# montyhall/bot7

Measured on NVIDIA B200. Metric: EI candidates scored/s at N=4096, S=32 hypers, higher is better.
Workload: dtype f64

## Files before the change

bot7_b200/csrc/api.cu:

```cuda
#include <math.h>
#include <stdarg.h>
#include <cmath>
#include <stdio.h>
#include <string.h>
#include <stdlib.h>

#include <algorithm>

#include "b7_internal.h"

static thread_local char g_err[512] = "";

void b7_set_error(const char* fmt, ...) {
  va_list ap;
  va_start(ap, fmt);
  vsnprintf(g_err, sizeof(g_err), fmt, ap);
  va_end(ap);
}

int b7_score_grid_size(b7_ctx* ctx, int64_t M);

namespace {

constexpr int kParStride = B7_MAX_DIMS + 4;
constexpr double kLog2Pi = 1.83787706640934548356;

constexpr size_t kCacheMin = (size_t)1 << 20;

void cache_flush(b7_ctx* ctx) {
  for (const b7_ctx::Block& b : ctx->cache) cudaFreeAsync(b.p, ctx->stream);
  ctx->cache.clear();
  ctx->cache_bytes = 0;
}

int dev_alloc_bytes(b7_ctx* ctx, void** p, size_t bytes) {
  *p = nullptr;
  bytes = (bytes + 255) / 256 * 256;
  if (bytes == 0) bytes = 256;
  if (bytes >= kCacheMin)
    for (size_t i = 0; i < ctx->cache.size(); ++i)
      if (ctx->cache[i].bytes == bytes) {
        *p = ctx->cache[i].p;
        ctx->cache_bytes -= bytes;
        ctx->cache[i] = ctx->cache.back();
        ctx->cache.pop_back();
        ctx->live[*p] = bytes;
        return 0;
      }
  cudaError_t e = cudaMallocFromPoolAsync(p, bytes, ctx->pool, ctx->stream);
  if (e != cudaSuccess && !ctx->cache.empty()) {
    cudaGetLastError();
    cache_flush(ctx);
    cudaStreamSynchronize(ctx->stream);
    cudaMemPoolTrimTo(ctx->pool, 0);
    e = cudaMallocFromPoolAsync(p, bytes, ctx->pool, ctx->stream);
  }
  if (e != cudaSuccess) {
    cudaGetLastError();
    b7_set_error("device allocation of %zu bytes failed: %s", bytes, cudaGetErrorString(e));
    return B7_ERR_NOMEM;
  }
  if (bytes >= kCacheMin) ctx->live[*p] = bytes;
  return 0;
}

template <typename T>
int dev_alloc(b7_ctx* ctx, T** p, size_t count) { return dev_alloc_bytes(ctx, (void**)p, (count ? count : 1) * sizeof(T)); }

inline void dev_free(b7_ctx* ctx, void* p) {
  if (!p) return;
  auto it = ctx->live.find(p);
  if (it != ctx->live.end()) {
    const size_t bytes = it->second;
    ctx->live.erase(it);
    if (ctx->cache_bytes + bytes <= ctx->cache_cap) {
      ctx->cache.push_back({p, bytes});
      ctx->cache_bytes += bytes;
      return;
    }
  }
  cudaFreeAsync(p, ctx->stream);
}

int grow(b7_ctx* ctx, double** p, size_t* have, size_t need_bytes) {
  if (*have >= need_bytes) return 0;
  dev_free(ctx, *p);
  *p = nullptr; *have = 0;
  B7_CHECK(dev_alloc(ctx, p, need_bytes / sizeof(double) + 1));
  *have = need_bytes;
  return 0;
}

inline int64_t pad128(int64_t n) { return (n + 127) / 128 * 128; }

inline int64_t panel_rows(b7_ctx* ctx, int Np = 4096) {
  const int64_t base = (int64_t)ctx->sm_count * 128;
  const int64_t f = Np >= 4096 ? 1 : std::min<int64_t>(8, 4096 / std::max(Np, 128));
  return base * f;
}

int sync_removed(b7_grid* g) {
  if (!g->removed_dirty) return 0;
  int64_t n = (int64_t)g->removed.size();
  if (n > g->removed_cap) {
    dev_free(g->ctx, g->removed_dev);
    g->removed_cap = std::max<int64_t>(256, 2 * n);
    B7_CHECK(dev_alloc(g->ctx, &g->removed_dev, (size_t)g->removed_cap));
  }
  if (n > 0)
    B7_CUDA(cudaMemcpyAsync(g->removed_dev, g->removed.data(), n * sizeof(int64_t), cudaMemcpyHostToDevice, g->ctx->stream));
  g->removed_dirty = false;
  return 0;
}

__device__ __forceinline__ long long tiled_index(int Np, int row, int k) {
  return ((long long)(row >> 7) * (Np >> 4) + (k >> 4)) * 2048 + ((k >> 2) & 3) * 512 + (row & 127) * 4 + (k & 3);
}

__global__ void frob_rows_kernel(const double* __restrict__ A, int Np, int N, double* __restrict__ out) {
  __shared__ double sh[256];
  double s = 0.0;
  const int row = blockIdx.x;
  for (int k = threadIdx.x; k <= row; k += blockDim.x) {
    const double v = A[tiled_index(Np, row, k)];
    s += (k < row ? 2.0 : 1.0) * v * v;
  }
  sh[threadIdx.x] = s;
  __syncthreads();
  for (int o = 128; o > 0; o >>= 1) {
    if (threadIdx.x < o) sh[threadIdx.x] += sh[threadIdx.x + o];
    __syncthreads();
  }
  if (threadIdx.x == 0) out[blockIdx.x] = sh[0];
}

__global__ void identity_kernel(double* __restrict__ A, int Np) {
  long long e = (long long)blockIdx.x * blockDim.x + threadIdx.x;
  if (e < (long long)Np * Np) { const int row = (int)(e / Np), k = (int)(e % Np); A[tiled_index(Np, row, k)] = (row == k) ? 1.0 : 0.0; }
}

int upload_residual(b7_gp* gp, int s, const std::vector<double>& yh) {
  std::vector<double> r((size_t)gp->Np, 0.0);
  const double m = gp->par_host[(size_t)s * kParStride + B7_MAX_DIMS + 2];
  for (int i = 0; i < gp->N; ++i) r[i] = yh[i] - m;
  B7_CUDA(cudaMemcpyAsync(gp->beta + (size_t)s * gp->Np, r.data(), gp->Np * sizeof(double), cudaMemcpyHostToDevice, gp->ctx->stream));
  B7_CUDA(cudaStreamSynchronize(gp->ctx->stream));
  return 0;
}

int build_kxx(b7_gp* gp, int s0, int count) {
  b7_ctx* ctx = gp->ctx;
  StageTimer t(ctx, ST_KBUILD);
  B7_CHECK(b7_launch_cov_batched(ctx, gp->kernel, gp->X, gp->N, gp->Np, gp->d, gp->Xt, gp->N, gp->Np,
                                 gp->par + (size_t)s0 * kParStride, kParStride, gp->fac + (size_t)s0 * gp->Np * gp->Np,
                                 (int64_t)gp->Np * gp->Np, count, true, true));
  t.stop(1);
  return 0;
}

int factor(b7_gp* gp, int s0, int count) {
  b7_ctx* ctx = gp->ctx;
  StageTimer t(ctx, ST_POTRF);
  int64_t before = ctx->launches;
  B7_CHECK(b7_launch_potrf(gp, s0, count));
  t.stop((int)(ctx->launches - before));
  return 0;
}

}

int b7_pool_alloc(b7_ctx* ctx, void** p, size_t bytes) {
  char* q = nullptr;
  int rc = dev_alloc(ctx, &q, bytes);
  *p = q;
  return rc;
}
void b7_pool_free(b7_ctx* ctx, void* p) { dev_free(ctx, p); }


extern "C" {

int b7_version(void) { return 100; }
const char* b7_last_error(void) { return g_err; }

int b7_device_count(void) {
  int n = 0;
  if (cudaGetDeviceCount(&n) != cudaSuccess) return 0;
  return n;
}

int b7_init(int device, b7_ctx** out) {
  if (!out) { b7_set_error("b7_init: out is null"); return B7_ERR_ARG; }
  *out = nullptr;
  int n = 0;
  cudaError_t e = cudaGetDeviceCount(&n);
  if (e != cudaSuccess || n == 0) {
    b7_set_error("b7_init: no CUDA device (%s); this library has no CPU path", e == cudaSuccess ? "count 0" : cudaGetErrorString(e));
    return B7_ERR_CUDA;
  }
  if (device < 0 || device >= n) { b7_set_error("b7_init: device %d out of range [0,%d)", device, n); return B7_ERR_ARG; }
  B7_CUDA(cudaSetDevice(device));
  b7_ctx* ctx = new b7_ctx();
  ctx->device = device;
  cudaDeviceProp p;
  B7_CUDA(cudaGetDeviceProperties(&p, device));
  ctx->sm_count = p.multiProcessorCount;
  if (p.major < 10) { b7_set_error("b7_init: device is sm_%d%d, this build is sm_100a only", p.major, p.minor); delete ctx; return B7_ERR_CUDA; }
  int prio_lo = 0, prio_hi = 0;
  B7_CUDA(cudaDeviceGetStreamPriorityRange(&prio_lo, &prio_hi));
  B7_CUDA(cudaStreamCreateWithPriority(&ctx->stream, cudaStreamNonBlocking, prio_hi));
  B7_CUDA(cudaStreamCreateWithPriority(&ctx->stream2, cudaStreamNonBlocking, prio_lo));
  B7_CUDA(cudaEventCreateWithFlags(&ctx->evA, cudaEventDisableTiming));
  B7_CUDA(cudaEventCreateWithFlags(&ctx->evB, cudaEventDisableTiming));
  B7_CUDA(cudaStreamCreateWithPriority(&ctx->stream3, cudaStreamNonBlocking, (prio_hi + prio_lo) / 2));
  B7_CUDA(cudaEventCreateWithFlags(&ctx->evS, cudaEventDisableTiming));
  B7_CUDA(cudaEventCreateWithFlags(&ctx->evS1, cudaEventDisableTiming));
  for (int i = 0; i < 2; ++i) {
    B7_CUDA(cudaEventCreateWithFlags(&ctx->evK[i], cudaEventDisableTiming));
    B7_CUDA(cudaEventCreateWithFlags(&ctx->evP[i], cudaEventDisableTiming));
  }
  { const char* e = getenv("B7_KSTAR_OVERLAP"); ctx->kstar_overlap = !(e && e[0] == '0'); }
  cudaMemPoolProps props = {};
  props.allocType = cudaMemAllocationTypePinned;
  props.handleTypes = cudaMemHandleTypeNone;
  props.location.type = cudaMemLocationTypeDevice;
  props.location.id = device;
  B7_CUDA(cudaMemPoolCreate(&ctx->pool, &props));
  unsigned long long keep = ~0ULL;
  B7_CUDA(cudaMemPoolSetAttribute(ctx->pool, cudaMemPoolAttrReleaseThreshold, &keep));
  {
    size_t free_b = 0, total_b = 0;
    B7_CUDA(cudaMemGetInfo(&free_b, &total_b));
    const char* e = getenv("B7_CACHE_FRACTION");
    const double frac = e ? atof(e) : 1.0 / 3.0;
    ctx->cache_cap = (size_t)((frac < 0.0 ? 0.0 : (frac > 0.9 ? 0.9 : frac)) * (double)total_b);
  }
  { const char* e = getenv("B7_POSTERIOR_I8"); ctx->use_i8 = !(e && e[0] == '0'); }
  { const char* e = getenv("B7_POTRF_I8"); ctx->potrf_i8 = !(e && e[0] == '0'); }
  { const char* e = getenv("B7_TRTRI_I8"); ctx->trtri_i8 = !(e && e[0] == '0'); }
  { const char* e = getenv("B7_POST_PAIR"); ctx->post_pair = !(e && e[0] == '0') && ctx->sm_count >= 2; }
  B7_CUDA(cudaEventCreate(&ctx->ev0));
  B7_CUDA(cudaEventCreate(&ctx->ev1));
  B7_CUDA(cudaEventCreate(&ctx->tm0));
  B7_CUDA(cudaEventCreate(&ctx->tm1));
  *out = ctx;
  return 0;
}

void b7_shutdown(b7_ctx* ctx) {
  if (!ctx) return;
  cudaSetDevice(ctx->device);
  cudaStreamSynchronize(ctx->stream);
  dev_free(ctx, ctx->ks);
  dev_free(ctx, ctx->moments);
  dev_free(ctx, ctx->xs_stage);
  dev_free(ctx, ctx->i8_partial);
  cache_flush(ctx);
  cudaStreamSynchronize(ctx->stream);
  cudaStreamSynchronize(ctx->stream2);
  cudaStreamSynchronize(ctx->stream3);
  cudaEventDestroy(ctx->evS);
  cudaEventDestroy(ctx->evS1);
  cudaStreamDestroy(ctx->stream3);
  cudaEventDestroy(ctx->evA);
  cudaEventDestroy(ctx->evB);
  for (int i = 0; i < 2; ++i) { cudaEventDestroy(ctx->evK[i]); cudaEventDestroy(ctx->evP[i]); }
  cudaStreamDestroy(ctx->stream2);
  cudaEventDestroy(ctx->ev0);
  cudaEventDestroy(ctx->ev1);
  cudaEventDestroy(ctx->tm0);
  cudaEventDestroy(ctx->tm1);
  cudaStreamDestroy(ctx->stream);
  if (ctx->pool) cudaMemPoolDestroy(ctx->pool);
  delete ctx;
}

int b7_sync(b7_ctx* ctx) {
  if (!ctx) return B7_ERR_ARG;
  B7_CUDA(cudaStreamSynchronize(ctx->stream));
  return 0;
}

int b7_set_posterior_path(b7_ctx* ctx, int path) {
  if (!ctx || (path != B7_PATH_FP64_DMMA && path != B7_PATH_INT8_OZAKI)) { b7_set_error("set_posterior_path: bad arguments"); return B7_ERR_ARG; }
  ctx->use_i8 = path == B7_PATH_INT8_OZAKI;
  return 0;
}
int b7_get_posterior_path(b7_ctx* ctx) { return ctx && ctx->use_i8 ? B7_PATH_INT8_OZAKI : B7_PATH_FP64_DMMA; }

int b7_timer_begin(b7_ctx* ctx) {
  if (!ctx) return B7_ERR_ARG;
  B7_CUDA(cudaSetDevice(ctx->device));
  B7_CUDA(cudaStreamSynchronize(ctx->stream));
  B7_CUDA(cudaEventRecord(ctx->tm0, ctx->stream));
  return 0;
}
int b7_timer_end(b7_ctx* ctx, double* ms) {
  if (!ctx || !ms) return B7_ERR_ARG;
  B7_CUDA(cudaEventRecord(ctx->tm1, ctx->stream));
  B7_CUDA(cudaEventSynchronize(ctx->tm1));
  float f = 0;
  B7_CUDA(cudaEventElapsedTime(&f, ctx->tm0, ctx->tm1));
  *ms = f;
  return 0;
}

int b7_set_profiling(b7_ctx* ctx, int on) { if (!ctx) return B7_ERR_ARG; ctx->profiling = on != 0; return 0; }
int b7_reset_stage_timers(b7_ctx* ctx) {
  if (!ctx) return B7_ERR_ARG;
  for (int i = 0; i < ST_COUNT; ++i) { ctx->stage_ms[i] = 0; ctx->stage_calls[i] = 0; }
  return 0;
}
int b7_last_stage_ms(b7_ctx* ctx, int stage, double* ms_total, int64_t* launches) {
  if (!ctx || stage < 0 || stage >= ST_COUNT) return B7_ERR_ARG;
  if (ms_total) *ms_total = ctx->stage_ms[stage];
  if (launches) *launches = ctx->stage_calls[stage];
  return 0;
}
int64_t b7_launch_count(b7_ctx* ctx) { return ctx ? ctx->launches : 0; }


int b7_sobol_directions(int dims, uint32_t* out) {
  if (dims < 1 || dims >= B7_MAX_DIMS || !out) { b7_set_error("sobol: dims must satisfy 1 <= dims < 40"); return B7_ERR_ARG; }
  b7_sobol_directions_host(dims, out);
  return 0;
}

int b7_sobol_generate(b7_ctx* ctx, int dims, int64_t first_seed, int64_t count, const double* mins,
                      const double* maxes, double* out_host, b7_grid** out_grid) {
  if (!ctx) return B7_ERR_ARG;
  if (out_grid) *out_grid = nullptr;
  if (dims < 1 || dims >= B7_MAX_DIMS) { b7_set_error("sobol: dims must satisfy 1 <= dims < 40"); return B7_ERR_ARG; }
  if (first_seed < 0) first_seed = 0;
  if (count < 0 || first_seed + count > (1LL << B7_SOBOL_BITS)) { b7_set_error("sobol: too many calls (seed range exceeds 2^30)"); return B7_ERR_ARG; }
  if ((mins == nullptr) != (maxes == nullptr)) { b7_set_error("sobol: one-sided rescaling is done by the host wrapper; pass both mins and maxes or neither"); return B7_ERR_ARG; }
  B7_CUDA(cudaSetDevice(ctx->device));
  double* dev = nullptr;
  B7_CHECK(dev_alloc(ctx, &dev, (size_t)count * dims));
  double *dmin = nullptr, *dscale = nullptr;
  if (mins) {
    double h[2 * B7_MAX_DIMS];
    for (int i = 0; i < dims; ++i) { h[i] = mins[i]; h[B7_MAX_DIMS + i] = maxes[i] + (-mins[i]); }
    B7_CHECK(dev_alloc(ctx, &dmin, 2 * B7_MAX_DIMS));
    dscale = dmin + B7_MAX_DIMS;
    B7_CUDA(cudaMemcpyAsync(dmin, h, sizeof(h), cudaMemcpyHostToDevice, ctx->stream));
    B7_CUDA(cudaStreamSynchronize(ctx->stream));
  }
  StageTimer t(ctx, ST_SOBOL);
  int rc = b7_launch_sobol(ctx, dims, first_seed, count, dmin, dscale, dev);
  t.stop(1);
  if (rc == 0 && out_host && count > 0) {
    cudaError_t e = cudaMemcpyAsync(out_host, dev, (size_t)count * dims * sizeof(double), cudaMemcpyDeviceToHost, ctx->stream);
    if (e != cudaSuccess) { b7_set_error("sobol D2H: %s", cudaGetErrorString(e)); rc = B7_ERR_CUDA; }
  }
  cudaError_t e = cudaStreamSynchronize(ctx->stream);
  if (rc == 0 && e != cudaSuccess) { b7_set_error("sobol: %s", cudaGetErrorString(e)); rc = B7_ERR_CUDA; }
  dev_free(ctx, dmin);
  if (rc != 0 || !out_grid) { dev_free(ctx, dev); return rc; }
  b7_grid* g = new b7_grid();
  g->ctx = ctx; g->rows = count; g->d = dims; g->X = dev;
  *out_grid = g;
  return 0;
}

int b7_grid_from_host(b7_ctx* ctx, const double* X, int64_t M, int d, b7_grid** out_grid) {
  if (!ctx || !out_grid || M < 0 || d < 1 || (M > 0 && !X)) { b7_set_error("grid_from_host: bad arguments"); return B7_ERR_ARG; }
  *out_grid = nullptr;
  B7_CUDA(cudaSetDevice(ctx->device));
  double* dev = nullptr;
  B7_CHECK(dev_alloc(ctx, &dev, (size_t)M * d));
  if (M > 0) {
    B7_CUDA(cudaMemcpyAsync(dev, X, (size_t)M * d * sizeof(double), cudaMemcpyHostToDevice, ctx->stream));
    B7_CUDA(cudaStreamSynchronize(ctx->stream));
  }
  b7_grid* g = new b7_grid();
  g->ctx = ctx; g->rows = M; g->d = d; g->X = dev;
  *out_grid = g;
  return 0;
}

int b7_grid_read(b7_grid* g, int64_t first_row, int64_t count, double* out_host) {
  if (!g || first_row < 0 || count < 0 || first_row + count > g->rows || (count > 0 && !out_host)) { b7_set_error("grid_read: range"); return B7_ERR_ARG; }
  B7_CUDA(cudaSetDevice(g->ctx->device));
  if (count == 0) return 0;
  B7_CUDA(cudaMemcpyAsync(out_host, g->X + first_row * g->d, (size_t)count * g->d * sizeof(double), cudaMemcpyDeviceToHost, g->ctx->stream));
  B7_CUDA(cudaStreamSynchronize(g->ctx->stream));
  return 0;
}

int64_t b7_grid_size(b7_grid* g) { return g ? g->rows - (int64_t)g->removed.size() : 0; }
int64_t b7_grid_rows(b7_grid* g) { return g ? g->rows : 0; }
int b7_grid_dims(b7_grid* g) { return g ? g->d : 0; }

static int64_t compacted_to_original(const b7_grid* g, int64_t c1) {
  int64_t r = c1 - 1;
  for (int64_t t : g->removed) {
    if (t <= r) ++r; else break;
  }
  return r;
}

int b7_grid_original_index(b7_grid* g, int64_t compacted_index, int64_t* original_index_1based) {
  if (!g || compacted_index < 1 || compacted_index > b7_grid_size(g)) { b7_set_error("grid: compacted index out of range"); return B7_ERR_ARG; }
  if (original_index_1based) *original_index_1based = compacted_to_original(g, compacted_index) + 1;
  return 0;
}

int b7_grid_remove(b7_grid* g, int64_t compacted_index, double* removed_row) {
  if (!g || compacted_index < 1 || compacted_index > b7_grid_size(g)) { b7_set_error("grid_remove: index out of range"); return B7_ERR_ARG; }
  int64_t r = compacted_to_original(g, compacted_index);
  if (removed_row) B7_CHECK(b7_grid_read(g, r, 1, removed_row));
  g->removed.insert(std::upper_bound(g->removed.begin(), g->removed.end(), r), r);
  g->removed_dirty = true;
  return 0;
}

void b7_grid_free(b7_grid* g) {
  if (!g) return;
  cudaSetDevice(g->ctx->device);
  dev_free(g->ctx, g->X);
  dev_free(g->ctx, g->removed_dev);
  delete g;
}


void b7_gp_free(b7_gp* gp) {
  if (!gp) return;
  cudaSetDevice(gp->ctx->device);
  cudaStreamSynchronize(gp->ctx->stream);
  void* ptrs[] = {gp->X, gp->Xt, gp->y, gp->par, gp->fac, gp->facS, gp->sigma, gp->dinv, gp->dinvT, gp->beta, gp->alpha, gp->tt, gp->logdet, gp->info, gp->meta_dev};
  for (void* p : ptrs) dev_free(gp->ctx, p);
  if (gp->potrf_graph) cudaGraphExecDestroy(gp->potrf_graph);
  delete gp;
}

int b7_gp_num_draws(b7_gp* gp) { return gp ? gp->S : 0; }
int b7_gp_num_obs(b7_gp* gp) { return gp ? gp->N : 0; }
int b7_gp_padded_n(b7_gp* gp) { return gp ? gp->Np : 0; }

static int gp_retry_draw(b7_gp* gp, int s, int first_info);

static void set_hypers_host(b7_gp* gp, const double* hyp) {
  const int d = gp->d, H = d + 3, S = gp->S;
  gp->par_host.assign((size_t)S * kParStride, 0.0);
  for (int s = 0; s < S; ++s) {
    const double* h = hyp + (size_t)s * H;
    double* p = gp->par_host.data() + (size_t)s * kParStride;
    for (int i = 0; i < d; ++i) p[i] = exp(-h[i]);
    const double sf2 = exp(2.0 * h[d]), sn2 = exp(2.0 * h[d + 1]);
    p[B7_MAX_DIMS] = sf2;
    p[B7_MAX_DIMS + 1] = sn2 + (gp->noiseless ? 1e-8 * sf2 : 0.0);
    p[B7_MAX_DIMS + 2] = h[d + 2];
    p[B7_MAX_DIMS + 3] = sn2;
  }
}

static void residuals_host(b7_gp* gp, const std::vector<double>& y, std::vector<double>& r) {
  r.assign((size_t)gp->S * gp->Np, 0.0);
  for (int s = 0; s < gp->S; ++s) {
    const double m = gp->par_host[(size_t)s * kParStride + B7_MAX_DIMS + 2];
    for (int i = 0; i < gp->N; ++i) r[(size_t)s * gp->Np + i] = y[i] - m;
  }
}

int b7_gp_fit_range(b7_gp* gp, int s0, int count, int* info, double* logml, double* jitter) {
  if (!gp || s0 < 0 || count < 0 || s0 + count > gp->S) { b7_set_error("gp_fit_range: draw range"); return B7_ERR_ARG; }
  b7_ctx* ctx = gp->ctx;
  B7_CUDA(cudaSetDevice(ctx->device));
  if (count == 0) return 0;
  B7_CHECK(build_kxx(gp, s0, count));
  B7_CHECK(factor(gp, s0, count));
  std::vector<int> inf((size_t)count);
  B7_CUDA(cudaMemcpyAsync(inf.data(), gp->info + s0, count * sizeof(int), cudaMemcpyDeviceToHost, ctx->stream));
  B7_CUDA(cudaStreamSynchronize(ctx->stream));
  for (int i = 0; i < count; ++i) {
    gp->jitter[s0 + i] = 0.0;
    gp->info_host[s0 + i] = 0;
    if (inf[i] != 0) B7_CHECK(gp_retry_draw(gp, s0 + i, inf[i]));
  }
  std::vector<double> bh((size_t)count * gp->Np), ldh((size_t)count);
  B7_CUDA(cudaMemcpyAsync(bh.data(), gp->beta + (size_t)s0 * gp->Np, bh.size() * sizeof(double), cudaMemcpyDeviceToHost, ctx->stream));
  B7_CUDA(cudaMemcpyAsync(ldh.data(), gp->logdet + s0, count * sizeof(double), cudaMemcpyDeviceToHost, ctx->stream));
  B7_CUDA(cudaStreamSynchronize(ctx->stream));
  for (int i = 0; i < count; ++i) {
    double q = 0.0;
    for (int k = 0; k < gp->N; ++k) q += bh[(size_t)i * gp->Np + k] * bh[(size_t)i * gp->Np + k];
    gp->logml_host[s0 + i] = -0.5 * q - ldh[i] - 0.5 * gp->N * kLog2Pi;
  }
  for (int i = 0; i < count; ++i) {
    if (info) info[i] = gp->info_host[s0 + i];
    if (logml) logml[i] = gp->logml_host[s0 + i];
    if (jitter) jitter[i] = gp->jitter[s0 + i];
  }
  return 0;
}

static int gp_retry_draw(b7_gp* gp, int s, int first_info) {
  b7_ctx* ctx = gp->ctx;
  const size_t fs = (size_t)gp->Np * gp->Np;
  double* par_s = gp->par + (size_t)s * kParStride;
  const double diag0 = gp->par_host[(size_t)s * kParStride + B7_MAX_DIMS + 1];
  B7_CHECK(build_kxx(gp, s, 1));
  double* rows = nullptr;
  B7_CHECK(dev_alloc(ctx, &rows, (size_t)gp->N));
  frob_rows_kernel<<<gp->N, 256, 0, ctx->stream>>>(gp->fac + s * fs, gp->Np, gp->N, rows);
  b7_count(ctx);
  std::vector<double> rh((size_t)gp->N);
  B7_CUDA(cudaMemcpyAsync(rh.data(), rows, gp->N * sizeof(double), cudaMemcpyDeviceToHost, ctx->stream));
  B7_CUDA(cudaStreamSynchronize(ctx->stream));
  dev_free(ctx, rows);
  double ss = 0.0;
  for (double v : rh) ss += v;
  const double max_eps = sqrt(ss);
  double eps = 1e-8;
  const double growth = 1.1;
  while (true) {
    if (eps > max_eps || !std::isfinite(max_eps)) {
      identity_kernel<<<(unsigned)((fs + 255) / 256), 256, 0, ctx->stream>>>(gp->fac + s * fs, gp->Np);
      b7_count(ctx);
      B7_CHECK(upload_residual(gp, s, gp->y_host));
      B7_CHECK(factor(gp, s, 1));
      gp->jitter[s] = INFINITY;
      gp->info_host[s] = first_info;
      return 0;
    }
    eps *= growth;
    double d = diag0 + eps;
    B7_CUDA(cudaMemcpyAsync(par_s + B7_MAX_DIMS + 1, &d, sizeof(double), cudaMemcpyHostToDevice, ctx->stream));
    B7_CUDA(cudaStreamSynchronize(ctx->stream));
    B7_CHECK(build_kxx(gp, s, 1));
    B7_CHECK(upload_residual(gp, s, gp->y_host));
    B7_CHECK(factor(gp, s, 1));
    int inf = 0;
    B7_CUDA(cudaMemcpyAsync(&inf, gp->info + s, sizeof(int), cudaMemcpyDeviceToHost, ctx->stream));
    B7_CUDA(cudaStreamSynchronize(ctx->stream));
    if (inf == 0) {
      gp->jitter[s] = eps;
      gp->info_host[s] = 0;
      B7_CUDA(cudaMemcpyAsync(par_s + B7_MAX_DIMS + 1, &diag0, sizeof(double), cudaMemcpyHostToDevice, ctx->stream));
      B7_CUDA(cudaStreamSynchronize(ctx->stream));
      return 0;
    }
  }
}

static bool i8_path(const b7_gp* gp) { return gp->ctx->use_i8 && gp->Np <= B7_I8_MAX_NP; }

static int gp_slice(b7_gp* gp, int s0, int count) {
  b7_ctx* ctx = gp->ctx;
  if (!gp->facS) {
    B7_CHECK(dev_alloc(ctx, &gp->facS, (size_t)gp->S * b7_i8_facs_stride(gp->Np)));
    B7_CHECK(dev_alloc(ctx, &gp->sigma, (size_t)gp->S * gp->Np));
  }
  B7_CHECK(b7_i8_slice_factor(ctx, gp->fac, gp->Np, gp->facS, gp->sigma, s0, count));
  for (int s = s0; s < s0 + count; ++s) gp->sliced[s] = 1;
  return 0;
}

static int gp_invert(b7_gp* gp, int s0, int count) {
  b7_ctx* ctx = gp->ctx;
  if (count <= 0) return 0;
  StageTimer t(ctx, ST_TRTRI);
  int64_t before = ctx->launches;
  if (gp->Np <= B7_I8_MAX_NP) B7_CHECK(b7_launch_alpha(gp, s0, count, false));
  B7_CHECK(b7_launch_trtri(gp, s0, count));
  for (int s = s0; s < s0 + count; ++s) gp->sliced[s] = 0;
  if (i8_path(gp)) B7_CHECK(gp_slice(gp, s0, count));
  t.stop((int)(ctx->launches - before));
  return 0;
}

int b7_gp_mark_ready(b7_gp* gp) {
  if (!gp) return B7_ERR_ARG;
  std::fill(gp->sliced.begin(), gp->sliced.end(), 0);
  if (i8_path(gp)) {
    B7_CUDA(cudaSetDevice(gp->ctx->device));
    B7_CHECK(b7_launch_alpha(gp, 0, gp->S, true));
    B7_CHECK(gp_slice(gp, 0, gp->S));
    B7_CUDA(cudaStreamSynchronize(gp->ctx->stream));
  }
  gp->ready = true;
  gp->inverted = true;
  return 0;
}

}

int b7_gp_prepare_gather(b7_gp* gp, int s0, int count) {
  b7_ctx* ctx = gp->ctx;
  B7_CUDA(cudaSetDevice(ctx->device));
  if (i8_path(gp) && !gp->facS) {
    B7_CHECK(dev_alloc(ctx, &gp->facS, (size_t)gp->S * b7_i8_facs_stride(gp->Np)));
    B7_CHECK(dev_alloc(ctx, &gp->sigma, (size_t)gp->S * gp->Np));
  }
  if (!gp->meta_dev) B7_CHECK(dev_alloc(ctx, &gp->meta_dev, (size_t)gp->S * 3));
  std::vector<double> m((size_t)std::max(count, 1) * 3);
  for (int i = 0; i < count; ++i) {
    m[3 * i] = (double)gp->info_host[s0 + i];
    m[3 * i + 1] = gp->logml_host[s0 + i];
    m[3 * i + 2] = gp->jitter[s0 + i];
  }
  if (count > 0) B7_CUDA(cudaMemcpyAsync(gp->meta_dev + 3 * (size_t)s0, m.data(), (size_t)count * 3 * sizeof(double), cudaMemcpyHostToDevice, ctx->stream));
  B7_CUDA(cudaStreamSynchronize(ctx->stream));
  return 0;
}

int b7_gp_finish_gather(b7_gp* gp, bool slices_exchanged) {
  b7_ctx* ctx = gp->ctx;
  B7_CUDA(cudaSetDevice(ctx->device));
  std::vector<double> m((size_t)gp->S * 3);
  B7_CUDA(cudaMemcpyAsync(m.data(), gp->meta_dev, m.size() * sizeof(double), cudaMemcpyDeviceToHost, ctx->stream));
  B7_CUDA(cudaStreamSynchronize(ctx->stream));
  for (int s = 0; s < gp->S; ++s) {
    gp->info_host[s] = (int)m[3 * s];
    gp->logml_host[s] = m[3 * s + 1];
    gp->jitter[s] = m[3 * s + 2];
  }
  std::fill(gp->sliced.begin(), gp->sliced.end(), slices_exchanged ? 1 : 0);
  gp->fac_complete = !slices_exchanged;
  gp->ready = true;
  gp->inverted = true;
  return 0;
}

extern "C" {

int b7_gp_fit(b7_ctx* ctx, int kernel, const double* X, const double* y, int N, int d, const double* hyp, int S,
              int H, int noiseless, int flags, b7_gp** out, int* info, double* logml, double* jitter) {
  if (!ctx || !out) { b7_set_error("gp_fit: null ctx/out"); return B7_ERR_ARG; }
  *out = nullptr;
  if (!X || !y || !hyp || N < 1 || d < 1 || d >= B7_MAX_DIMS || S < 1 || H != d + 3 ||
      (kernel != B7_KERNEL_ARDSE && kernel != B7_KERNEL_MATERN52)) {
    b7_set_error("gp_fit: bad arguments (N=%d d=%d S=%d H=%d kernel=%d; H must be d+3, d < 40)", N, d, S, H, kernel);
    return B7_ERR_ARG;
  }
  B7_CUDA(cudaSetDevice(ctx->device));
  b7_gp* gp = new b7_gp();
  gp->ctx = ctx; gp->kernel = kernel; gp->N = N; gp->d = d; gp->S = S; gp->noiseless = noiseless;
  gp->Np = (int)pad128(N); gp->NB = gp->Np / B7_NB;
  gp->jitter.assign(S, 0.0); gp->info_host.assign(S, 0); gp->logml_host.assign(S, 0.0); gp->sliced.assign(S, 0);
  const size_t Np = gp->Np, fs = Np * Np, ds = (size_t)gp->NB * B7_NB * B7_NB;
  int rc = 0;
  auto fail = [&](int code) { b7_gp_free(gp); return code; };
  if ((rc = dev_alloc(ctx, &gp->X, (size_t)N * d)) || (rc = dev_alloc(ctx, &gp->Xt, (size_t)d * Np)) || (rc = dev_alloc(ctx, &gp->y, (size_t)N)) ||
      (rc = dev_alloc(ctx, &gp->par, (size_t)S * kParStride)) || (rc = dev_alloc(ctx, &gp->fac, (size_t)S * fs)) ||
      (rc = dev_alloc(ctx, &gp->dinv, (size_t)S * ds)) || (rc = dev_alloc(ctx, &gp->dinvT, (size_t)S * ds)) ||
      (rc = dev_alloc(ctx, &gp->beta, (size_t)S * Np)) || (rc = dev_alloc(ctx, &gp->alpha, (size_t)S * Np)) ||
      (rc = dev_alloc(ctx, &gp->tt, (size_t)S * B7_NB * Np)) ||
      (rc = dev_alloc(ctx, &gp->logdet, (size_t)S)) || (rc = dev_alloc(ctx, &gp->info, (size_t)S)))
    return fail(rc);
  if (cudaMemsetAsync(gp->dinv, 0, (size_t)S * ds * sizeof(double), ctx->stream) != cudaSuccess) return fail(B7_ERR_CUDA);
  gp->y_host.assign(y, y + N);
  set_hypers_host(gp, hyp);
  std::vector<double> xt((size_t)d * Np, 0.0), r;
  for (int i = 0; i < N; ++i)
    for (int k = 0; k < d; ++k) xt[(size_t)k * Np + i] = X[(size_t)i * d + k];
  residuals_host(gp, gp->y_host, r);
  cudaStream_t st = ctx->stream;
  cudaError_t e;
  if ((e = cudaMemcpyAsync(gp->X, X, (size_t)N * d * sizeof(double), cudaMemcpyHostToDevice, st)) != cudaSuccess ||
      (e = cudaMemcpyAsync(gp->Xt, xt.data(), xt.size() * sizeof(double), cudaMemcpyHostToDevice, st)) != cudaSuccess ||
      (e = cudaMemcpyAsync(gp->y, y, (size_t)N * sizeof(double), cudaMemcpyHostToDevice, st)) != cudaSuccess ||
      (e = cudaMemcpyAsync(gp->par, gp->par_host.data(), gp->par_host.size() * sizeof(double), cudaMemcpyHostToDevice, st)) != cudaSuccess ||
      (e = cudaMemcpyAsync(gp->beta, r.data(), r.size() * sizeof(double), cudaMemcpyHostToDevice, st)) != cudaSuccess ||
      (e = cudaStreamSynchronize(st)) != cudaSuccess) {
    b7_set_error("gp_fit upload: %s", cudaGetErrorString(e));
    return fail(B7_ERR_CUDA);
  }
  if (flags == B7_FIT_DEFER) { *out = gp; return 0; }
  if ((rc = b7_gp_fit_range(gp, 0, S, info, logml, jitter)) < 0) return fail(rc);
  if (flags == B7_FIT_PREDICT) {
    if ((rc = gp_invert(gp, 0, S)) < 0) return fail(rc);
    gp->inverted = true;
  }
  if ((e = cudaStreamSynchronize(st)) != cudaSuccess) { b7_set_error("gp_fit: %s", cudaGetErrorString(e)); return fail(B7_ERR_CUDA); }
  gp->ready = true;
  *out = gp;
  return 0;
}

int b7_gp_refit(b7_gp* gp, const double* hyp, int flags, int* info, double* logml, double* jitter) {
  if (!gp || !hyp || (flags != B7_FIT_PREDICT && flags != B7_FIT_LOGML_ONLY)) { b7_set_error("gp_refit: bad arguments"); return B7_ERR_ARG; }
  b7_ctx* ctx = gp->ctx;
  B7_CUDA(cudaSetDevice(ctx->device));
  set_hypers_host(gp, hyp);
  std::vector<double> r;
  residuals_host(gp, gp->y_host, r);
  gp->ready = false; gp->inverted = false;
  B7_CUDA(cudaMemcpyAsync(gp->par, gp->par_host.data(), gp->par_host.size() * sizeof(double), cudaMemcpyHostToDevice, ctx->stream));
  B7_CUDA(cudaMemcpyAsync(gp->beta, r.data(), r.size() * sizeof(double), cudaMemcpyHostToDevice, ctx->stream));
  B7_CUDA(cudaStreamSynchronize(ctx->stream));
  B7_CHECK(b7_gp_fit_range(gp, 0, gp->S, info, logml, jitter));
  if (flags == B7_FIT_PREDICT) {
    B7_CHECK(gp_invert(gp, 0, gp->S));
    gp->inverted = true;
  }
  B7_CUDA(cudaStreamSynchronize(ctx->stream));
  gp->ready = true;
  return 0;
}

int b7_gp_invert_range(b7_gp* gp, int s0, int count) {
  if (!gp || s0 < 0 || count < 0 || s0 + count > gp->S) return B7_ERR_ARG;
  B7_CUDA(cudaSetDevice(gp->ctx->device));
  B7_CHECK(gp_invert(gp, s0, count));
  B7_CUDA(cudaStreamSynchronize(gp->ctx->stream));
  return 0;
}

int b7_gp_device_ptr(b7_gp* gp, int what, void** ptr, int64_t* bytes) {
  if (!gp || !ptr) return B7_ERR_ARG;
  const int64_t Np = gp->Np;
  switch (what) {
    case 0: *ptr = gp->fac; if (bytes) *bytes = (int64_t)gp->S * Np * Np * 8; return 0;
    case 1: *ptr = gp->beta; if (bytes) *bytes = (int64_t)gp->S * Np * 8; return 0;
    case 2: *ptr = gp->dinv; if (bytes) *bytes = (int64_t)gp->S * gp->NB * B7_NB * B7_NB * 8; return 0;
    default: b7_set_error("gp_device_ptr: what=%d", what); return B7_ERR_ARG;
  }
}

int b7_gp_read_factor(b7_gp* gp, int s, double* out_host) {
  if (!gp || !out_host || s < 0 || s >= gp->S) return B7_ERR_ARG;
  B7_CUDA(cudaSetDevice(gp->ctx->device));
  double* tmp = nullptr;
  B7_CHECK(dev_alloc(gp->ctx, &tmp, (size_t)gp->N * gp->N));
  int rc = b7_launch_untile(gp->ctx, gp->fac + (size_t)s * gp->Np * gp->Np, tmp, gp->Np, gp->N);
  cudaError_t e = cudaMemcpyAsync(out_host, tmp, (size_t)gp->N * gp->N * 8, cudaMemcpyDeviceToHost, gp->ctx->stream);
  if (e == cudaSuccess) e = cudaStreamSynchronize(gp->ctx->stream);
  dev_free(gp->ctx, tmp);
  if (rc < 0) return rc;
  if (e != cudaSuccess) { b7_set_error("gp_read_factor: %s", cudaGetErrorString(e)); return B7_ERR_CUDA; }
  return 0;
}

static int posterior_panel(b7_gp* gp, int s, const double* A, int64_t rows, double* mean, double* var) {
  b7_ctx* ctx = gp->ctx;
  const int64_t rp = pad128(rows);
  B7_CHECK(grow(ctx, &ctx->ks, &ctx->ks_bytes, (size_t)rp * gp->Np * 8));
  const double* p = gp->par_host.data() + (size_t)s * kParStride;
  if (!gp->fac_complete && (!i8_path(gp) || !gp->sliced[s])) {
    b7_set_error("gp: this handle came from a sharded fit that exchanged the int8 slices only; refit to use the FP64 path");
    return B7_ERR_STATE;
  }
  if (i8_path(gp)) {
    if (!gp->sliced[s]) B7_CHECK(gp_slice(gp, s, 1));
    int e = 0;
    frexp(p[B7_MAX_DIMS], &e);
    const double tau = ldexp(1.0, e);
    const int64_t rp64 = (rows + 63) / 64 * 64;
    int8_t* ksS = reinterpret_cast<int8_t*>(ctx->ks);
    B7_CHECK(grow(ctx, &ctx->i8_partial, &ctx->i8_partial_bytes, b7_i8_partial_bytes(gp->Np, rp64)));
    {
      StageTimer t(ctx, ST_KSTAR);
      B7_CHECK(b7_i8_cov_slices(ctx, ctx->stream, gp->kernel, A, rows, rp64, gp->d, gp->Xt, gp->N, gp->Np, gp->par + (size_t)s * kParStride, tau,
                                gp->alpha + (size_t)s * gp->Np, ksS, b7_i8_mean_partials(ctx->i8_partial, gp->Np, rp64)));
      t.stop(1);
    }
    StageTimer t(ctx, ST_POSTERIOR);
    B7_CHECK(b7_launch_posterior_i8(ctx, gp->facS + (size_t)s * b7_i8_facs_stride(gp->Np), gp->sigma + (size_t)s * gp->Np, gp->Np, ksS, A, rows,
                                    gp->d, gp->Xt, gp->par + (size_t)s * kParStride, gp->kernel, rp64, tau, p[B7_MAX_DIMS], p[B7_MAX_DIMS + 2],
                                    ctx->i8_partial, mean, var));
    t.stop(1);
    return 0;
  }
  {
    StageTimer t(ctx, ST_KSTAR);
    B7_CHECK(b7_launch_cov_batched(ctx, gp->kernel, A, rows, rp, gp->d, gp->Xt, gp->N, gp->Np,
                                   gp->par + (size_t)s * kParStride, 0, ctx->ks, 0, 1, false, true));
    t.stop(1);
  }
  {
    StageTimer t(ctx, ST_POSTERIOR);
    B7_CHECK(b7_launch_posterior(ctx, gp->fac + (size_t)s * gp->Np * gp->Np, gp->beta + (size_t)s * gp->Np, gp->Np, ctx->ks,
                                 rp, p[B7_MAX_DIMS], p[B7_MAX_DIMS + 2], mean, var));
    t.stop(1);
  }
  return 0;
}

static int posterior_panel_draws_i8(b7_gp* gp, const double* A, int64_t rows, double* dm, double* dv, int64_t ld) {
  b7_ctx* ctx = gp->ctx;
  const int S = gp->S;
  const int64_t rp64 = (rows + 63) / 64 * 64;
  const size_t ks_bytes = ((size_t)rp64 * gp->Np * B7_I8_SLICES + 255) / 256 * 256;
  const size_t part_bytes = (b7_i8_partial_bytes(gp->Np, rp64) + 255) / 256 * 256;
  B7_CHECK(grow(ctx, &ctx->ks, &ctx->ks_bytes, 2 * ks_bytes));
  B7_CHECK(grow(ctx, &ctx->i8_partial, &ctx->i8_partial_bytes, 2 * part_bytes));
  for (int s = 0; s < S; ++s)
    if (!gp->sliced[s]) B7_CHECK(gp_slice(gp, s, 1));
  auto tau_of = [&](int s) {
    int e = 0;
    frexp(gp->par_host[(size_t)s * kParStride + B7_MAX_DIMS], &e);
    return ldexp(1.0, e);
  };
  auto ks_of = [&](int s) { return reinterpret_cast<int8_t*>(ctx->ks) + (size_t)(s & 1) * ks_bytes; };
  auto part_of = [&](int s) { return reinterpret_cast<double*>(reinterpret_cast<char*>(ctx->i8_partial) + (size_t)(s & 1) * part_bytes); };
  auto kstar = [&](int s) {
    return b7_i8_cov_slices(ctx, ctx->stream2, gp->kernel, A, rows, rp64, gp->d, gp->Xt, gp->N, gp->Np, gp->par + (size_t)s * kParStride, tau_of(s),
                            gp->alpha + (size_t)s * gp->Np, ks_of(s), b7_i8_mean_partials(part_of(s), gp->Np, rp64));
  };
  B7_CUDA(cudaEventRecord(ctx->evA, ctx->stream));
  B7_CUDA(cudaStreamWaitEvent(ctx->stream2, ctx->evA, 0));
  B7_CHECK(kstar(0));
  B7_CUDA(cudaEventRecord(ctx->evK[0], ctx->stream2));
  for (int s = 0; s < S; ++s) {
    if (s + 1 < S) {
      if (s >= 1) B7_CUDA(cudaStreamWaitEvent(ctx->stream2, ctx->evP[(s + 1) & 1], 0));
      B7_CHECK(kstar(s + 1));
      B7_CUDA(cudaEventRecord(ctx->evK[(s + 1) & 1], ctx->stream2));
    }
    B7_CUDA(cudaStreamWaitEvent(ctx->stream, ctx->evK[s & 1], 0));
    const double* p = gp->par_host.data() + (size_t)s * kParStride;
    B7_CHECK(b7_launch_posterior_i8(ctx, gp->facS + (size_t)s * b7_i8_facs_stride(gp->Np), gp->sigma + (size_t)s * gp->Np, gp->Np, ks_of(s), A, rows,
                                    gp->d, gp->Xt, gp->par + (size_t)s * kParStride, gp->kernel, rp64, tau_of(s), p[B7_MAX_DIMS], p[B7_MAX_DIMS + 2],
                                    part_of(s), dm + (size_t)s * ld, dv + (size_t)s * ld));
    B7_CUDA(cudaEventRecord(ctx->evP[s & 1], ctx->stream));
  }
  return 0;
}

static bool all_sliced_or_sliceable(const b7_gp* gp) {
  if (gp->fac_complete) return true;
  for (char c : gp->sliced) if (!c) return false;
  return true;
}

static int require_predict_state(b7_gp* gp) {
  if (!gp->ready || !gp->inverted) {
    b7_set_error("gp: factor not inverted (fit with B7_FIT_PREDICT, or b7_gp_invert_range + b7_gp_mark_ready)");
    return B7_ERR_STATE;
  }
  return 0;
}

int b7_gp_predict(b7_gp* gp, int s, const double* Xs, int64_t M, double* mean, double* var) {
  if (!gp || s < 0 || s >= gp->S || M < 0 || (M > 0 && (!Xs || !mean || !var))) { b7_set_error("gp_predict: bad arguments"); return B7_ERR_ARG; }
  B7_CHECK(require_predict_state(gp));
  b7_ctx* ctx = gp->ctx;
  B7_CUDA(cudaSetDevice(ctx->device));
  const int64_t P = panel_rows(ctx, gp->Np);
  B7_CHECK(grow(ctx, &ctx->xs_stage, &ctx->xs_bytes, (size_t)std::min(P, pad128(M)) * gp->d * 8));
  B7_CHECK(grow(ctx, &ctx->moments, &ctx->moments_bytes, (size_t)2 * std::min(P, pad128(M)) * 8));
  for (int64_t c0 = 0; c0 < M; c0 += P) {
    const int64_t n = std::min(P, M - c0), np = pad128(n);
    B7_CUDA(cudaMemcpyAsync(ctx->xs_stage, Xs + c0 * gp->d, (size_t)n * gp->d * 8, cudaMemcpyHostToDevice, ctx->stream));
    double* dm = ctx->moments; double* dv = ctx->moments + np;
    B7_CHECK(posterior_panel(gp, s, ctx->xs_stage, n, dm, dv));
    B7_CUDA(cudaMemcpyAsync(mean + c0, dm, (size_t)n * 8, cudaMemcpyDeviceToHost, ctx->stream));
    B7_CUDA(cudaMemcpyAsync(var + c0, dv, (size_t)n * 8, cudaMemcpyDeviceToHost, ctx->stream));
    B7_CUDA(cudaStreamSynchronize(ctx->stream));
  }
  return 0;
}


struct PartBuf {
  b7_ctx* ctx = nullptr;
  double* best = nullptr; int64_t* idx = nullptr; int64_t* nan = nullptr; int cap = 0;
  explicit PartBuf(b7_ctx* c) : ctx(c) {}
  ~PartBuf() { dev_free(ctx, best); dev_free(ctx, idx); dev_free(ctx, nan); }
};

static int finish_argmax(b7_ctx* ctx, PartBuf& pb, int n_parts, double* best, int64_t* row0based, int64_t* nan_count) {
  std::vector<double> hb((size_t)n_parts); std::vector<int64_t> hi((size_t)n_parts), hn((size_t)n_parts);
  if (n_parts > 0) {
    B7_CUDA(cudaMemcpyAsync(hb.data(), pb.best, n_parts * 8, cudaMemcpyDeviceToHost, ctx->stream));
    B7_CUDA(cudaMemcpyAsync(hi.data(), pb.idx, n_parts * 8, cudaMemcpyDeviceToHost, ctx->stream));
    B7_CUDA(cudaMemcpyAsync(hn.data(), pb.nan, n_parts * 8, cudaMemcpyDeviceToHost, ctx->stream));
  }
  B7_CUDA(cudaStreamSynchronize(ctx->stream));
  double bv = -INFINITY; int64_t bi = INT64_MAX, nn = 0;
  for (int p = 0; p < n_parts; ++p) {
    nn += hn[p];
    if (hi[p] == INT64_MAX) continue;
    if (hb[p] > bv || (hb[p] == bv && hi[p] < bi)) { bv = hb[p]; bi = hi[p]; }
  }
  if (bi == INT64_MAX) { *best = NAN; *row0based = -1; } else { *best = bv; *row0based = bi; }
  *nan_count = nn;
  return 0;
}

int b7_acq_score_range(b7_gp* gp, b7_grid* grid, int64_t row0, int64_t count, int kind, double tradeoff, int bound,
                       double sign, double fmin, double* score_host, int64_t* argmax_original, double* best,
                       int64_t* nan_count) {
  if (!gp || !grid || row0 < 0 || count < 0 || row0 + count > grid->rows || grid->d != gp->d ||
      (kind != B7_SCORE_EI && kind != B7_SCORE_CB)) {
    b7_set_error("acq_score: bad arguments (grid dims %d vs model dims %d)", grid ? grid->d : -1, gp ? gp->d : -1);
    return B7_ERR_ARG;
  }
  if (grid->ctx != gp->ctx) { b7_set_error("acq_score: the grid and the model live on different contexts / devices"); return B7_ERR_ARG; }
  B7_CHECK(require_predict_state(gp));
  b7_ctx* ctx = gp->ctx;
  B7_CUDA(cudaSetDevice(ctx->device));
  B7_CHECK(sync_removed(grid));
  const int64_t P = panel_rows(ctx, gp->Np), Pp = std::min(P, pad128(std::max<int64_t>(count, 1)));
  const int S = gp->S;
  B7_CHECK(grow(ctx, &ctx->moments, &ctx->moments_bytes, (size_t)2 * S * Pp * 8));
  const int64_t n_panels = (count + P - 1) / P;
  PartBuf pb(ctx);
  pb.cap = (int)(n_panels * b7_score_grid_size(ctx, P)) + 1;
  B7_CHECK(dev_alloc(ctx, &pb.best, (size_t)pb.cap)); B7_CHECK(dev_alloc(ctx, &pb.idx, (size_t)pb.cap)); B7_CHECK(dev_alloc(ctx, &pb.nan, (size_t)pb.cap));
  struct ScoreBuf { b7_ctx* c; double* p; ~ScoreBuf() { dev_free(c, p); } } sb{ctx, nullptr};
  if (score_host) B7_CHECK(dev_alloc(ctx, &sb.p, (size_t)std::max<int64_t>(count, 1)));
  double* const score_dev = sb.p;
  int n_parts = 0, rc = 0;
  for (int64_t c0 = 0; c0 < count && rc == 0; c0 += P) {
    const int64_t n = std::min(P, count - c0), np = pad128(n);
    double* dm = ctx->moments; double* dv = ctx->moments + (size_t)S * np;
    if (i8_path(gp) && ctx->kstar_overlap && !ctx->profiling && S > 1 && all_sliced_or_sliceable(gp))
      rc = posterior_panel_draws_i8(gp, grid->X + (row0 + c0) * grid->d, n, dm, dv, np);
    else
      for (int s = 0; s < S && rc == 0; ++s)
        rc = posterior_panel(gp, s, grid->X + (row0 + c0) * grid->d, n, dm + (size_t)s * np, dv + (size_t)s * np);
    if (rc < 0) break;
    StageTimer t(ctx, ST_SCORE);
    int parts = 0;
    rc = b7_launch_score(ctx, kind, dm, dv, S, n, np, tradeoff, bound, sign, fmin, grid->removed_dev,
                         (int64_t)grid->removed.size(), row0 + c0, score_dev ? score_dev + c0 : nullptr, pb.best + n_parts,
                         pb.idx + n_parts, pb.nan + n_parts, &parts);
    t.stop(1);
    n_parts += parts;
  }
  double bv = NAN; int64_t r0 = -1, nn = 0;
  if (rc == 0) rc = finish_argmax(ctx, pb, n_parts, &bv, &r0, &nn);
  if (rc == 0 && score_host && count > 0) {
    cudaError_t e = cudaMemcpyAsync(score_host, score_dev, (size_t)count * 8, cudaMemcpyDeviceToHost, ctx->stream);
    if (e == cudaSuccess) e = cudaStreamSynchronize(ctx->stream);
    if (e != cudaSuccess) { b7_set_error("acq_score D2H: %s", cudaGetErrorString(e)); rc = B7_ERR_CUDA; }
  }
  if (rc < 0) return rc;
  if (argmax_original) *argmax_original = r0 + 1;
  if (best) *best = bv;
  if (nan_count) *nan_count = nn;
  return 0;
}

int b7_acq_score(b7_gp* gp, b7_grid* grid, int kind, double tradeoff, int bound, double sign, double fmin,
                 double* score_host, int64_t* argmax, int64_t* argmax_original, double* best, int64_t* nan_count) {
  if (!grid) { b7_set_error("acq_score: null grid"); return B7_ERR_ARG; }
  int64_t orig = 0;
  B7_CHECK(b7_acq_score_range(gp, grid, 0, grid->rows, kind, tradeoff, bound, sign, fmin, score_host, &orig, best, nan_count));
  if (argmax_original) *argmax_original = orig;
  if (argmax) {
    if (orig <= 0) *argmax = 0;
    else {
      int64_t r = orig - 1;
      int64_t below = std::lower_bound(grid->removed.begin(), grid->removed.end(), r) - grid->removed.begin();
      *argmax = r - below + 1;
    }
  }
  return 0;
}

int b7_score_moments(b7_ctx* ctx, int kind, const double* mean, const double* var, int S, int64_t M, double tradeoff,
                     int bound, double sign, double fmin, double* score_host, int64_t* argmax, double* best,
                     int64_t* nan_count) {
  if (!ctx || S < 1 || M < 0 || (M > 0 && (!mean || !var)) || (kind != B7_SCORE_EI && kind != B7_SCORE_CB)) { b7_set_error("score_moments: bad arguments"); return B7_ERR_ARG; }
  B7_CUDA(cudaSetDevice(ctx->device));
  const size_t n = (size_t)S * std::max<int64_t>(M, 1);
  double *dm = nullptr, *dv = nullptr, *ds = nullptr;
  B7_CHECK(dev_alloc(ctx, &dm, n)); B7_CHECK(dev_alloc(ctx, &dv, n)); B7_CHECK(dev_alloc(ctx, &ds, (size_t)std::max<int64_t>(M, 1)));
  PartBuf pb(ctx); pb.cap = b7_score_grid_size(ctx, M) + 1;
  B7_CHECK(dev_alloc(ctx, &pb.best, (size_t)pb.cap)); B7_CHECK(dev_alloc(ctx, &pb.idx, (size_t)pb.cap)); B7_CHECK(dev_alloc(ctx, &pb.nan, (size_t)pb.cap));
  int rc = 0, parts = 0;
  if (M > 0) {
    B7_CUDA(cudaMemcpyAsync(dm, mean, (size_t)S * M * 8, cudaMemcpyHostToDevice, ctx->stream));
    B7_CUDA(cudaMemcpyAsync(dv, var, (size_t)S * M * 8, cudaMemcpyHostToDevice, ctx->stream));
    StageTimer t(ctx, ST_SCORE);
    rc = b7_launch_score(ctx, kind, dm, dv, S, M, M, tradeoff, bound, sign, fmin, nullptr, 0, 0, ds, pb.best, pb.idx, pb.nan, &parts);
    t.stop(1);
  }
  double bv = NAN; int64_t r0 = -1, nn = 0;
  if (rc == 0) rc = finish_argmax(ctx, pb, parts, &bv, &r0, &nn);
  if (rc == 0 && score_host && M > 0) {
    cudaError_t e = cudaMemcpyAsync(score_host, ds, (size_t)M * 8, cudaMemcpyDeviceToHost, ctx->stream);
    if (e == cudaSuccess) e = cudaStreamSynchronize(ctx->stream);
    if (e != cudaSuccess) { b7_set_error("score_moments D2H: %s", cudaGetErrorString(e)); rc = B7_ERR_CUDA; }
  }
  dev_free(ctx, dm); dev_free(ctx, dv); dev_free(ctx, ds);
  if (rc < 0) return rc;
  if (argmax) *argmax = r0 + 1;
  if (best) *best = bv;
  if (nan_count) *nan_count = nn;
  return 0;
}

}
```

bot7_b200/csrc/b7_internal.h:

```cpp
#pragma once
#include <cuda_runtime.h>
#include <stdint.h>
#include <string>
#include <unordered_map>
#include <vector>

#include "../../include/bot7_b200.h"

#define B7_NB 128
#define B7_MAX_DIMS 40
#define B7_SOBOL_BITS 30

void b7_set_error(const char* fmt, ...);

#define B7_CUDA(expr)                                                                              \
  do {                                                                                             \
    cudaError_t e_ = (expr);                                                                       \
    if (e_ != cudaSuccess) {                                                                       \
      b7_set_error("CUDA error %s at %s:%d (%s)", cudaGetErrorString(e_), __FILE__, __LINE__, #expr); \
      return B7_ERR_CUDA;                                                                          \
    }                                                                                              \
  } while (0)

#define B7_CHECK(expr)                 \
  do {                                 \
    int rc_ = (expr);                  \
    if (rc_ < 0) return rc_;           \
  } while (0)

enum { ST_SOBOL = 0, ST_KBUILD, ST_POTRF, ST_TRTRI, ST_KSTAR, ST_POSTERIOR, ST_SCORE, ST_BLR, ST_COUNT };

struct b7_ctx {
  int device = 0;
  int sm_count = 148;
  cudaStream_t stream = nullptr;
  cudaMemPool_t pool = nullptr;
  cudaStream_t stream2 = nullptr;
  cudaStream_t stream3 = nullptr;
  cudaEvent_t evA = nullptr, evB = nullptr, evS = nullptr, evS1 = nullptr;
  cudaEvent_t evK[2] = {nullptr, nullptr}, evP[2] = {nullptr, nullptr};
  bool kstar_overlap = true;
  cudaEvent_t ev0 = nullptr, ev1 = nullptr, tm0 = nullptr, tm1 = nullptr;
  double stage_ms[ST_COUNT] = {0};
  int64_t stage_calls[ST_COUNT] = {0};
  bool profiling = false;
  bool use_i8 = false;
  bool potrf_i8 = true;
  bool trtri_i8 = true;
  bool post_pair = true;
  int64_t launches = 0;
  double* ks = nullptr;
  size_t ks_bytes = 0;
  double* moments = nullptr;
  size_t moments_bytes = 0;
  double* xs_stage = nullptr;
  size_t xs_bytes = 0;
  double* i8_partial = nullptr;
  size_t i8_partial_bytes = 0;
  struct Block { void* p; size_t bytes; };
  std::vector<Block> cache;
  std::unordered_map<void*, size_t> live;
  size_t cache_bytes = 0, cache_cap = 0;
};

struct b7_grid {
  b7_ctx* ctx = nullptr;
  int64_t rows = 0;
  int d = 0;
  double* X = nullptr;
  std::vector<int64_t> removed;
  int64_t* removed_dev = nullptr;
  int64_t removed_cap = 0;
  bool removed_dirty = false;
  int64_t row_base = 0, rows_total = 0;
  std::vector<int64_t> removed_global;
};

struct b7_gp {
  b7_ctx* ctx = nullptr;
  int kernel = 0, N = 0, d = 0, S = 0, Np = 0, NB = 0, DT = 8, noiseless = 0;
  bool inverted = false, ready = false;
  double* X = nullptr;
  double* Xt = nullptr;
  double* y = nullptr;
  double* par = nullptr;
  std::vector<double> par_host;
  std::vector<double> y_host;
  double* fac = nullptr;
  int8_t* facS = nullptr;
  double* alpha = nullptr;
  double* sigma = nullptr;
  double* dinv = nullptr;
  double* dinvT = nullptr;
  double* beta = nullptr;
  double* tt = nullptr;
  double* logdet = nullptr;
  int* info = nullptr;
  double* meta_dev = nullptr;
  cudaGraphExec_t potrf_graph = nullptr;
  int potrf_graph_s0 = -1, potrf_graph_count = 0, potrf_graph_launches = 0, potrf_calls_s0 = -1, potrf_calls_count = 0, potrf_calls = 0;
  bool fac_complete = true;
  std::vector<char> sliced;
  std::vector<double> jitter;
  std::vector<int> info_host;
  std::vector<double> logml_host;
};

struct b7_blr {
  b7_ctx* ctx = nullptr;
  int N = 0, D = 0, S = 0;
  double* Linv = nullptr;
  double* w = nullptr;
  double* par = nullptr;
  std::vector<double> par_host;
  bool ready = true;
  double* Z = nullptr;
  double* y = nullptr;
  double* partial = nullptr;
  int gram_blocks = 0;
  double* gram = nullptr;
  double* hyp = nullptr;
  double* ev_w = nullptr;
  double* ev_stat = nullptr;
  double* ev_res = nullptr;
  double* ev_out = nullptr;
  int* ev_info = nullptr;
};

int b7_gp_prepare_gather(b7_gp* gp, int s0, int count);
int b7_gp_finish_gather(b7_gp* gp, bool slices_exchanged);
bool b7_dngo_tiles_fit(int n_layers, const int* dims, int D);
int b7_check_act(const char* what, int n_layers, const int* act);
inline std::vector<int> b7_relu_codes(int n_layers, int relu_last) {
  std::vector<int> act((size_t)(n_layers > 0 ? n_layers : 1), B7_ACT_RELU);
  if (n_layers > 0 && !relu_last) act[(size_t)n_layers - 1] = B7_ACT_NONE;
  return act;
}

int b7_pool_alloc(b7_ctx* ctx, void** p, size_t bytes);
void b7_pool_free(b7_ctx* ctx, void* p);

static inline void b7_count(b7_ctx* ctx, int n = 1) { ctx->launches += n; }
struct StageTimer {
  b7_ctx* ctx; int stage;
  StageTimer(b7_ctx* c, int s) : ctx(c), stage(s) { if (ctx->profiling) cudaEventRecord(ctx->ev0, ctx->stream); }
  void stop(int n = 1) {
    if (!ctx->profiling) return;
    cudaEventRecord(ctx->ev1, ctx->stream);
    cudaEventSynchronize(ctx->ev1);
    float ms = 0; cudaEventElapsedTime(&ms, ctx->ev0, ctx->ev1);
    ctx->stage_ms[stage] += ms;
    ctx->stage_calls[stage] += n;
  }
};

void b7_sobol_directions_host(int dims, uint32_t* out );
int b7_launch_sobol(b7_ctx* ctx, int dims, int64_t first_seed, int64_t count, const double* mins_dev,
                    const double* maxes_dev, double* out_dev);
int b7_launch_cov_batched(b7_ctx* ctx, int kernel, const double* A , int64_t rows, int64_t rows_pad, int d,
                          const double* Xt , int N, int Np, const double* par, int64_t par_stride,
                          double* out , int64_t out_stride, int batch, bool is_kxx, bool tiled = false);
int b7_launch_potrf(b7_gp* gp, int s0, int count);
int b7_launch_trtri(b7_gp* gp, int s0, int count);
int b7_launch_alpha(b7_gp* gp, int s0, int count, bool from_inverse);
int b7_launch_untile(b7_ctx* ctx, const double* facT, double* out , int Np, int N);
int b7_launch_posterior(b7_ctx* ctx, const double* LinvT , const double* beta, int Np, const double* ksT ,
                        int64_t cols_pad, double sf2, double mconst, double* mean, double* var);
size_t b7_i8_panel_bytes(int Np, int W);
int b7_i8_panel_slice(b7_ctx* ctx, cudaStream_t st, const double* fac, int Np, int kb0, int kb1, int row0_blk, int8_t* pA, int8_t* pB,
                      size_t p_stride, double* sig, int s0, int count);
int b7_i8_trail(b7_ctx* ctx, cudaStream_t st, double* fac, int Np, const int8_t* pA, const int8_t* pB, size_t p_stride, const double* sig,
                int kb0, int kb1, int row0_blk, int it0, int n_it, int nt0, int n_nt, int s0, int count);
int b7_launch_trtri_i8(b7_gp* gp, int s0, int count);
#define B7_I8_SLICES 7
#define B7_I8_MAX_NP 16384
size_t b7_i8_facs_stride(int Np);
int b7_i8_slice_factor(b7_ctx* ctx, const double* fac, int Np, int8_t* facS, double* sigma, int s0, int count);
int b7_i8_cov_slices(b7_ctx* ctx, cudaStream_t st, int kernel, const double* A, int64_t rows, int64_t rows_pad, int d, const double* Xt,
                     int N, int Np, const double* par, double tau, const double* alpha, int8_t* ksS, double* meanP);
int b7_launch_posterior_i8(b7_ctx* ctx, const int8_t* facS, const double* sigma, int Np, const int8_t* ksS, const double* cand,
                           int64_t rows, int d, const double* Xt, const double* par, int kernel, int64_t cols_pad, double tau,
                           double sf2, double mconst, double* partial, double* mean, double* var);
size_t b7_i8_partial_bytes(int Np, int64_t cols_pad);
double* b7_i8_mean_partials(double* partial, int Np, int64_t cols_pad);
int b7_launch_score(b7_ctx* ctx, int kind, const double* mean, const double* var, int S, int64_t M, int64_t ld,
                    double tradeoff, int bound, double sign, double fmin, const int64_t* removed, int64_t n_removed,
                    int64_t row_base, double* score_out , double* part_best, int64_t* part_idx,
                    int64_t* part_nan, int* n_parts);
int b7_argmax_finish(b7_ctx* ctx, const double* part_best, const int64_t* part_idx, const int64_t* part_nan,
                     int n_parts, double* best, int64_t* idx0, int64_t* nan_count);
```

bot7_b200/csrc/posterior_i8.cu:

```cuda
#include <math.h>
#include <stdlib.h>

#include "b7_internal.h"
#include "exp_neg.cuh"
#include "gemm_tile.cuh"
#include "i8_common.cuh"

using b7g::mbar_init; using b7g::mbar_wait; using b7g::mbar_arrive; using b7g::mbar_arrive_expect_tx; using b7g::bulk_g2s;
using b7g::mbar_fence_init; using b7g::smem_u32;
using namespace b7i8;

namespace {

constexpr int TM = 128, TN = 64, KB = 64;
constexpr int KC = KB / 16;
constexpr int A_STAGE = NS * TM * KB;
constexpr int B_STAGE = NS * TN * KB;
constexpr int STAGE = A_STAGE + B_STAGE;
constexpr int NSTAGE = 2;
static_assert(STAGE % 1024 == 0 && KB % 32 == 0 && 64 % KB == 0, "stage geometry");
static_assert(KB == b7i8::gemm::KB && TM == b7i8::gemm::TM && TN == b7i8::gemm::TN && NSTAGE == b7i8::gemm::NSTAGE,
              "posterior_i8_kernel issues its MMAs through the shared stage of i8_common.cuh");
constexpr int I8_THREADS = 192;
constexpr int RED_BYTES = 2 * 4 * TN * 8;
constexpr int I8_SMEM = NSTAGE * STAGE + RED_BYTES + 1024;
constexpr int TNH = TN / 2;
constexpr int B_HALF = NS * TNH * KB;
constexpr int P_STAGE = A_STAGE + B_HALF;
constexpr int P_NSTAGE = 3;
constexpr int P_SMEM = P_NSTAGE * P_STAGE + RED_BYTES + 1024;
constexpr int P_THREADS = 320;
static_assert(P_STAGE % 1024 == 0 && P_SMEM <= 227 * 1024, "pair stage geometry");


__host__ __device__ __forceinline__ long long pk_off(int rb) {
  const long long j = rb >> 1;
  return 4 * j * (j + 1) + (rb & 1) * 4 * (j + 1);
}

__global__ void __launch_bounds__(SLICE_THREADS)
slice_factor_kernel(const double* __restrict__ fac, long long fac_stride, int Np, int8_t* __restrict__ facS,
                    long long facS_stride, double* __restrict__ sigma, int s0) {
  __shared__ double s_red[SLICE_THREADS];
  const int rb = blockIdx.x, s = s0 + blockIdx.y, row = threadIdx.x & 127, q = threadIdx.x >> 7;
  const int KTA = Np / 16, NB = Np / TM;
  const int n_kc = rb < NB ? (rb + 1) * (TM / 16) : 0, all_kc = ((rb >> 1) + 1) * 4 * KC;
  int8_t* dst = facS + (long long)s * facS_stride + pk_off(rb) * A_STAGE;
  double inv = 0.0;
  const double* src = fac + (long long)s * fac_stride + b7g::tile_off(KTA, rb < NB ? rb : 0, 0);
  if (rb < NB) {
    double mx = 0.0;
    bool bad = false;
    for (int kc = q; kc < n_kc; kc += 4) chunk_max(src + b7g::elem_off(row, kc * 16), mx, bad);
    const double sg = row_scale(mx, bad, s_red, row, q);
    inv = sg != sg ? 0.0 : 1.0 / sg;
    if (q == 0) sigma[(long long)s * Np + rb * TM + row] = sg;
  }
  for (int kc = q; kc < all_kc; kc += 4) {
    uint32_t pk[4][NS];
    if (kc < n_kc) {
      chunk_digits(src + b7g::elem_off(row, kc * 16), inv, pk);
    } else {
#pragma unroll
      for (int g = 0; g < 4; ++g)
#pragma unroll
        for (int p = 0; p < NS; ++p) pk[g][p] = 0u;
    }
    const int ks = kc / KC, kcc = kc % KC;
#pragma unroll
    for (int p = 0; p < NS; ++p)
      *reinterpret_cast<uint4*>(dst + (long long)ks * A_STAGE + p * (KC * TM * 16) + kcc * (TM * 16) + row * 16) =
          make_uint4(pk[0][p], pk[1][p], pk[2][p], pk[3][p]);
  }
}

template <int DT, int KERNEL, bool PAIR>
__global__ void __launch_bounds__(128)
cov_slices_kernel(const double* __restrict__ A, long long rows, int d, const double* __restrict__ Xt, int N, int Np,
                  const double* __restrict__ par, double inv_tau, const double* __restrict__ alpha, int8_t* __restrict__ ksS,
                  double* __restrict__ meanP) {
  __shared__ __align__(16) double s_x[DT][64];
  __shared__ double s_w[DT];
  __shared__ double s_tab[64];
  __shared__ __align__(16) double s_al[64];
  __shared__ double s_dot[64];
  if (threadIdx.x < 64) s_tab[threadIdx.x] = c_exp_tab[threadIdx.x];
  const int ct = blockIdx.x, kb64 = blockIdx.y, KS_ALL = Np / KB;
  const int c = threadIdx.x & 63;
  for (int e = threadIdx.x; e < DT * 64; e += 128) {
    const int i = e / 64, k = kb64 * 64 + e % 64;
    s_x[i][e % 64] = (i < d && k < N) ? Xt[(long long)i * Np + k] : 0.0;
  }
  if (threadIdx.x >= 64) s_al[c] = alpha[kb64 * 64 + c];
  if (threadIdx.x < DT) s_w[threadIdx.x] = threadIdx.x < d ? par[threadIdx.x] : 0.0;
  __syncthreads();
  const long long row = (long long)ct * TN + c;
  double a[DT];
#pragma unroll
  for (int i = 0; i < DT; ++i) a[i] = (row < rows && i < d) ? A[row * d + i] : 0.0;
  const double sf2s = par[B7_MAX_DIMS] * inv_tau * 18014398509481984.0;
  double dot = 0.0;
  double w[DT];
#pragma unroll
  for (int j = 0; j < DT; ++j) w[j] = s_w[j];
  ExpNegK K;
  K.init();
  const bool live = row < rows;
#pragma unroll 1
  for (int half = 0; half < 2; ++half) {
  const int kc = (threadIdx.x >> 6) + 2 * half;
  uint32_t pk[4][NS];
  unsigned long long z[4];
#pragma unroll
  for (int i = 0; i < 16; i += 2) {
    const int kk = kc * 16 + i, k = kb64 * 64 + kk;
    double r2a = 0.0, r2b = 0.0;
#pragma unroll
    for (int j = 0; j < DT; ++j) {
      const double2 x2 = *reinterpret_cast<const double2*>(&s_x[j][kk]);
      const double ta = (a[j] - x2.x) * w[j], tb = (a[j] - x2.y) * w[j];
      r2a = fma(ta, ta, r2a);
      r2b = fma(tb, tb, r2b);
    }
    double va, vb;
    if (KERNEL == B7_KERNEL_ARDSE) {
      va = sf2s * exp_neg_k(-0.5 * r2a, s_tab, K);
      vb = sf2s * exp_neg_k(-0.5 * r2b, s_tab, K);
    } else {
      const double ra = sqrt(r2a), s5a = 2.23606797749978969641 * ra, rb = sqrt(r2b), s5b = 2.23606797749978969641 * rb;
      va = sf2s * ((1.0 + s5a + (5.0 / 3.0) * r2a) * exp_neg_k(-s5a, s_tab, K));
      vb = sf2s * ((1.0 + s5b + (5.0 / 3.0) * r2b) * exp_neg_k(-s5b, s_tab, K));
    }
    va = (live && k < N) ? va : 0.0;
    vb = (live && k + 1 < N) ? vb : 0.0;
    const double2 al = *reinterpret_cast<const double2*>(&s_al[kk]);
    dot = fma(va, al.x, dot);
    dot = fma(vb, al.y, dot);
    z[i & 3] = digit_bytes_scaled(va);
    z[(i & 3) + 1] = digit_bytes_scaled(vb);
    if ((i & 3) == 2) pack4(z, pk[i >> 2]);
  }
  const int gkc = kb64 * 4 + kc, ks = gkc / KC, kcc = gkc % KC;
  int8_t* dst = PAIR ? ksS + (((long long)ct * KS_ALL + ks) * 2 + (c >> 5)) * B_HALF + kcc * (TNH * 16) + (c & 31) * 16
                     : ksS + ((long long)ct * KS_ALL + ks) * B_STAGE + kcc * (TN * 16) + c * 16;
  constexpr int P_STRIDE = PAIR ? KC * TNH * 16 : KC * TN * 16;
#pragma unroll
  for (int p = 0; p < NS; ++p) *reinterpret_cast<uint4*>(dst + p * P_STRIDE) = make_uint4(pk[0][p], pk[1][p], pk[2][p], pk[3][p]);
  }
  if (threadIdx.x >= 64) s_dot[c] = dot;
  __syncthreads();
  if (threadIdx.x < 64) meanP[((long long)ct * (Np / 64) + kb64) * 64 + c] = dot + s_dot[c];
}

__device__ __forceinline__ double lane_transpose_sum(double (&x)[32], int lane) {
#pragma unroll
  for (int s = 16; s >= 1; s >>= 1) {
    const bool up = (lane & s) != 0;
#pragma unroll
    for (int j = 0; j < s; ++j) {
      const double send = up ? x[j] : x[j + s];
      const double keep = up ? x[j + s] : x[j];
      x[j] = keep + __shfl_xor_sync(0xffffffffu, send, s);
    }
  }
  return x[0];
}

struct Walk {
  int NB, chunk, group, n_tiles;
  __device__ __forceinline__ int cpt() const { return (NB + chunk - 1) / chunk; }
  __device__ __forceinline__ int npl() const { return (cpt() + 1) / 2; }
  __device__ __forceinline__ int n_items() const { return n_tiles * npl(); }
  __device__ __forceinline__ int grp(int item) const {
    const int g = item / (group * npl()), last = (n_tiles - 1) / group;
    return g < last ? g : last;
  }
  __device__ __forceinline__ int g_tiles(int g) const { return n_tiles - g * group < group ? n_tiles - g * group : group; }
  __device__ __forceinline__ int tile(int item) const {
    const int g = grp(item);
    return g * group + (item - g * group * npl()) % g_tiles(g);
  }
  __device__ __forceinline__ int level(int item) const {
    const int g = grp(item);
    return (item - g * group * npl()) / g_tiles(g);
  }
  __device__ __forceinline__ int parts(int item) const { return 2 * level(item) == cpt() - 1 ? 1 : 2; }
  __device__ __forceinline__ int rb_begin(int item, int part) const { return (part == 0 ? level(item) : cpt() - 1 - level(item)) * chunk; }
  __device__ __forceinline__ int rb_end(int item, int part) const {
    const int e = rb_begin(item, part) + chunk;
    return e < NB ? e : NB;
  }
};


template <typename F>
__device__ __forceinline__ void epilogue_row_block(uint32_t tmem, int tid, int warp, int lane, double sc, double* rr, double* out,
                                                   F arrive_drained) {
  double v[TN];
  b7i8::gemm::drain_classes(tmem, warp, v);
  tc_fence_before();
  __syncwarp();
  if (lane == 0) arrive_drained();
#pragma unroll
  for (int h = 0; h < 2; ++h) {
    double x[32];
#pragma unroll
    for (int c = 0; c < 32; ++c) { const double vv = v[h * 32 + c] * sc; x[c] = vv * vv; }
    rr[warp * TN + h * 32 + lane] = lane_transpose_sum(x, lane);
  }
  asm volatile("bar.sync 1, 128;\n" ::: "memory");
  if (tid < TN && out) out[tid] = ((rr[0 * TN + tid] + rr[1 * TN + tid]) + rr[2 * TN + tid]) + rr[3 * TN + tid];
}

template <typename F>
__device__ __forceinline__ void epilogue_row_block8(uint32_t tmem, int tid, int warp, int lane, double sc, double* rr, double* out,
                                                    F arrive_drained) {
  const int q = warp & 3, hc = warp >> 2;
  const uint32_t base = tmem + ((uint32_t)(q * 32) << 16) + (uint32_t)(hc * 32);
  double v[32];
  uint32_t a[4][32];
#pragma unroll
  for (int i = 0; i < 3; ++i) tmem_ld32_async(base + (uint32_t)(i * TN), a[i]);
  tmem_ld_wait();
#pragma unroll
  for (int c = 0; c < 32; ++c) v[c] = 0.0;
#pragma unroll
  for (int i = 0; i < 3; ++i) {
    tmem_pin(a[i]);
    const double wt = ldexp(1.0, 4 - 8 * (i + 2));
#pragma unroll
    for (int c = 0; c < 32; ++c) v[c] = fma((double)(int)a[i][c], wt, v[c]);
  }
#pragma unroll
  for (int i = 0; i < 4; ++i) tmem_ld32_async(base + (uint32_t)((3 + i) * TN), a[i]);
  tmem_ld_wait();
#pragma unroll
  for (int i = 0; i < 4; ++i) tmem_pin(a[i]);
  tc_fence_before();
  __syncwarp();
  if (lane == 0) arrive_drained();
#pragma unroll
  for (int i = 0; i < 4; ++i) {
    const double wt = ldexp(1.0, 4 - 8 * (i + 5));
#pragma unroll
    for (int c = 0; c < 32; ++c) v[c] = fma((double)(int)a[i][c], wt, v[c]);
  }
#pragma unroll
  for (int c = 0; c < 32; ++c) { const double vv = v[c] * sc; v[c] = vv * vv; }
  rr[q * TN + hc * 32 + lane] = lane_transpose_sum(v, lane);
  asm volatile("bar.sync 1, 256;\n" ::: "memory");
  if (tid < TN && out) out[tid] = ((rr[0 * TN + tid] + rr[1 * TN + tid]) + rr[2 * TN + tid]) + rr[3 * TN + tid];
}

__global__ void __launch_bounds__(I8_THREADS, 1)
posterior_i8_kernel(const int8_t* __restrict__ facS, const double* __restrict__ sigma, int Np, int NB,
                    const int8_t* __restrict__ ksS, double tau, int chunk, int group, int n_tiles, double* __restrict__ partial) {
  extern __shared__ __align__(1024) uint8_t smem[];
  double* red = reinterpret_cast<double*>(smem + NSTAGE * STAGE);
  uint64_t* bars = reinterpret_cast<uint64_t*>(smem + NSTAGE * STAGE + RED_BYTES);
  uint64_t *full = bars, *empty = bars + NSTAGE, *acc_full = bars + 2 * NSTAGE, *acc_empty = bars + 2 * NSTAGE + 1;
  uint32_t* tmem_slot = reinterpret_cast<uint32_t*>(bars + 2 * NSTAGE + 2);
  const int tid = threadIdx.x, warp = tid >> 5, lane = tid & 31;
  const int KS_ALL = Np / KB;
  const Walk wk{NB, chunk, group, n_tiles};
  if (tid == 0) {
    for (int s = 0; s < NSTAGE; ++s) { mbar_init(full + s, 1); mbar_init(empty + s, 1); }
    mbar_init(acc_full, 1);
    mbar_init(acc_empty, 4);
    mbar_fence_init();
  }
  if (warp == 4) {
    asm volatile("tcgen05.alloc.cta_group::1.sync.aligned.shared::cta.b32 [%0], %1;\n" ::"r"(smem_u32(tmem_slot)), "n"(512) : "memory");
    asm volatile("tcgen05.relinquish_alloc_permit.cta_group::1.sync.aligned;\n" ::: "memory");
  }
  tc_fence_before();
  __syncthreads();
  tc_fence_after();
  const uint32_t tmem = *tmem_slot;

  if (warp == 4) {
    int slot = 0;
    unsigned phase = 1;
    bool wrapped = false;
    for (int item = blockIdx.x; item < wk.n_items(); item += gridDim.x) {
      const int tile = wk.tile(item);
      const int8_t* gB = ksS + (long long)tile * KS_ALL * B_STAGE;
      for (int part = 0; part < wk.parts(item); ++part)
        for (int rb = wk.rb_begin(item, part); rb < wk.rb_end(item, part); ++rb) {
          const int8_t* gA = facS + pk_off(rb) * A_STAGE;
          for (int ks = 0; ks < (TM / KB) * (rb + 1); ++ks) {
            if (wrapped) mbar_wait(empty + slot, phase);
            if (elect_one()) {
              uint8_t* st = smem + slot * STAGE;
              mbar_arrive_expect_tx(full + slot, STAGE);
              bulk_g2s(st, gA + (long long)ks * A_STAGE, A_STAGE, full + slot);
              bulk_g2s(st + A_STAGE, gB + (long long)ks * B_STAGE, B_STAGE, full + slot);
            }
            __syncwarp();
            if (++slot == NSTAGE) { slot = 0; phase ^= 1u; wrapped = true; }
          }
        }
    }
  } else if (warp == 5) {
    const uint32_t idesc = (2u << 4) | (1u << 7) | (1u << 10) | ((uint32_t)(TN >> 3) << 17) | ((uint32_t)(TM >> 4) << 24);
    int slot = 0, done = 0;
    unsigned phase = 0;
    for (int item = blockIdx.x; item < wk.n_items(); item += gridDim.x)
      for (int part = 0; part < wk.parts(item); ++part)
        for (int rb = wk.rb_begin(item, part); rb < wk.rb_end(item, part); ++rb, ++done) {
          if (done > 0) { mbar_wait(acc_empty, (unsigned)((done - 1) & 1)); tc_fence_after(); }
          const int n_ks = (TM / KB) * (rb + 1);
          for (int ks = 0; ks < n_ks; ++ks) {
            mbar_wait(full + slot, phase);
            tc_fence_after();
            if (elect_one()) {
              b7i8::gemm::mma_stage(smem + slot * STAGE, tmem, idesc, ks == 0);
              umma_commit(empty + slot);
              if (ks == n_ks - 1) umma_commit(acc_full);
            }
            __syncwarp();
            if (++slot == NSTAGE) { slot = 0; phase ^= 1u; }
          }
        }
  } else {
    int done = 0;
    for (int item = blockIdx.x; item < wk.n_items(); item += gridDim.x) {
      const int tile = wk.tile(item);
      for (int part = 0; part < wk.parts(item); ++part)
        for (int rb = wk.rb_begin(item, part); rb < wk.rb_end(item, part); ++rb, ++done) {
          mbar_wait(acc_full, (unsigned)(done & 1));
          tc_fence_after();
          epilogue_row_block(tmem, tid, warp, lane, sigma[rb * TM + tid] * tau, red + (done & 1) * (4 * TN),
                             partial + ((long long)tile * NB + rb) * TN, [&] { mbar_arrive(acc_empty); });
        }
    }
  }
  tc_fence_before();
  __syncthreads();
  if (warp == 4) asm volatile("tcgen05.dealloc.cta_group::1.sync.aligned.b32 %0, %1;\n" ::"r"(tmem), "n"(512) : "memory");
}

__global__ void __cluster_dims__(2, 1, 1) __launch_bounds__(P_THREADS, 1)
posterior_i8_pair_kernel(const int8_t* __restrict__ facS, const double* __restrict__ sigma, int Np, int NB,
                         const int8_t* __restrict__ ksS, double tau, int group, int n_tiles, double* __restrict__ partial, int dbg) {
  extern __shared__ __align__(1024) uint8_t smem[];
  double* red = reinterpret_cast<double*>(smem + P_NSTAGE * P_STAGE);
  uint64_t* bars = reinterpret_cast<uint64_t*>(smem + P_NSTAGE * P_STAGE + RED_BYTES);
  uint64_t *full = bars, *empty = bars + P_NSTAGE, *peer_full = bars + 2 * P_NSTAGE, *acc_full = bars + 3 * P_NSTAGE,
           *acc_empty = bars + 3 * P_NSTAGE + 1;
  uint32_t* tmem_slot = reinterpret_cast<uint32_t*>(bars + 3 * P_NSTAGE + 2);
  const int tid = threadIdx.x, warp = tid >> 5, lane = tid & 31;
  const int KS_ALL = Np / KB;
  const uint32_t rank = cluster_ctarank();
  const int pair_id = blockIdx.x >> 1, n_pairs = gridDim.x >> 1;
  const Walk wk{(NB + 1) / 2, 1, group, n_tiles};
  if (tid == 0) {
    for (int s = 0; s < P_NSTAGE; ++s) { mbar_init(full + s, 1); mbar_init(empty + s, 1); mbar_init(peer_full + s, 1); }
    mbar_init(acc_full, 1);
    mbar_init(acc_empty, 16);
    mbar_fence_init();
  }
  if (warp == 8) {
    asm volatile("tcgen05.alloc.cta_group::2.sync.aligned.shared::cta.b32 [%0], %1;\n" ::"r"(smem_u32(tmem_slot)), "n"(512) : "memory");
    asm volatile("tcgen05.relinquish_alloc_permit.cta_group::2.sync.aligned;\n" ::: "memory");
  }
  tc_fence_before();
  __syncthreads();
  cluster_sync_all();
  tc_fence_after();
  const uint32_t tmem = *tmem_slot;

  if (warp == 8) {
    const uint64_t pol_last = l2_policy_evict_last(), pol_first = l2_policy_evict_first();
    int slot = 0;
    unsigned phase = 1;
    bool wrapped = false;
    for (int item = pair_id; item < wk.n_items(); item += n_pairs) {
      const int tile = wk.tile(item);
      const int8_t* gB = ksS + ((long long)tile * KS_ALL * 2 + rank) * B_HALF;
      for (int part = 0; part < wk.parts(item); ++part)
        for (int j = wk.rb_begin(item, part); j < wk.rb_end(item, part); ++j) {
          const int8_t* gA = facS + pk_off(2 * j + (int)rank) * A_STAGE;
          for (int ks = 0; ks < 4 * (j + 1); ++ks) {
            if (wrapped) mbar_wait_cluster(empty + slot, phase);
            if (elect_one()) {
              uint8_t* st = smem + slot * P_STAGE;
              if (dbg & 4) {
                mbar_arrive_expect_tx(full + slot, 2048);
                bulk_g2s(st, facS, 1024, full + slot);
                bulk_g2s(st + A_STAGE, ksS, 1024, full + slot);
                __syncwarp();
                if (++slot == P_NSTAGE) { slot = 0; phase ^= 1u; wrapped = true; }
                continue;
              }
              mbar_arrive_expect_tx(full + slot, P_STAGE);
              if (dbg & 2) {
                bulk_g2s(st, facS, A_STAGE, full + slot);
                bulk_g2s(st + A_STAGE, ksS, B_HALF, full + slot);
              } else {
                const int hint = dbg >> 4;
                if (hint == 1 || hint == 2) bulk_g2s_hint(st, gA + (long long)ks * A_STAGE, A_STAGE, full + slot, pol_last);
                else if (hint == 4 || hint == 5) bulk_g2s_hint(st, gA + (long long)ks * A_STAGE, A_STAGE, full + slot, pol_first);
                else bulk_g2s(st, gA + (long long)ks * A_STAGE, A_STAGE, full + slot);
                if (hint == 2 || hint == 3) bulk_g2s_hint(st + A_STAGE, gB + (long long)ks * (2 * B_HALF), B_HALF, full + slot, pol_first);
                else if (hint == 4 || hint == 6) bulk_g2s_hint(st + A_STAGE, gB + (long long)ks * (2 * B_HALF), B_HALF, full + slot, pol_last);
                else bulk_g2s(st + A_STAGE, gB + (long long)ks * (2 * B_HALF), B_HALF, full + slot);
              }
            }
            __syncwarp();
            if (++slot == P_NSTAGE) { slot = 0; phase ^= 1u; wrapped = true; }
          }
        }
    }
  } else if (warp == 9) {
    int slot = 0, done = 0;
    unsigned phase = 0;
    if (rank == 0) {
      const uint32_t idesc = (2u << 4) | (1u << 7) | (1u << 10) | ((uint32_t)(TN >> 3) << 17) | ((uint32_t)(256 >> 4) << 24);
      for (int item = pair_id; item < wk.n_items(); item += n_pairs)
        for (int part = 0; part < wk.parts(item); ++part)
          for (int j = wk.rb_begin(item, part); j < wk.rb_end(item, part); ++j, ++done) {
            if (done > 0) { mbar_wait_cluster(acc_empty, (unsigned)((done - 1) & 1)); tc_fence_after(); }
            const int n_ks = 4 * (j + 1);
            for (int ks = 0; ks < n_ks; ++ks) {
              mbar_wait_cluster(full + slot, phase);
              mbar_wait_cluster(peer_full + slot, phase);
              tc_fence_after();
              if (elect_one()) {
                const uint8_t* st = smem + slot * P_STAGE;
                const uint64_t da0 = umma_desc(st, TM * 16, 128), db0 = umma_desc(st + A_STAGE, TNH * 16, 128);
#pragma unroll
                for (int k2 = 0; k2 < KB / 32; ++k2) {
#pragma unroll
                  for (int p = 1; p <= NS; ++p) {
                    const uint64_t da = da0 + (uint64_t)(((p - 1) * (KC * TM * 16) + k2 * (2 * TM * 16)) >> 4);
                    const uint32_t acc = (ks == 0 && k2 == 0 && p == 1) ? 0u : 1u;
                    const int nq = NS + 1 - p;
#pragma unroll
                    for (int q = 1; q <= nq; ++q) {
                      const uint64_t db = db0 + (uint64_t)(((q - 1) * (KC * TNH * 16) + k2 * (2 * TNH * 16)) >> 4);
                      const uint32_t dcol = tmem + (uint32_t)((p + q - 2) * TN);
                      if (nq == 1) umma_i8_pair<0>(dcol, da, db, idesc, acc);
                      else if (q == 1) umma_i8_pair<1>(dcol, da, db, idesc, acc);
                      else if (q == nq) umma_i8_pair<3>(dcol, da, db, idesc, acc);
                      else umma_i8_pair<2>(dcol, da, db, idesc, acc);
                    }
                  }
                }
                umma_commit_pair(empty + slot);
                if (ks == n_ks - 1) umma_commit_pair(acc_full);
              }
              __syncwarp();
              if (++slot == P_NSTAGE) { slot = 0; phase ^= 1u; }
            }
          }
    } else {
      for (int item = pair_id; item < wk.n_items(); item += n_pairs)
        for (int part = 0; part < wk.parts(item); ++part)
          for (int j = wk.rb_begin(item, part); j < wk.rb_end(item, part); ++j)
            for (int ks = 0; ks < 4 * (j + 1); ++ks) {
              mbar_wait_cluster(full + slot, phase);
              if (elect_one()) mbar_arrive_cluster(peer_full + slot, 0);
              __syncwarp();
              if (++slot == P_NSTAGE) { slot = 0; phase ^= 1u; }
            }
    }
  } else {
    int done = 0;
    for (int item = pair_id; item < wk.n_items(); item += n_pairs) {
      const int tile = wk.tile(item);
      for (int part = 0; part < wk.parts(item); ++part)
        for (int j = wk.rb_begin(item, part); j < wk.rb_end(item, part); ++j, ++done) {
          const int rb = 2 * j + (int)rank;
          mbar_wait_cluster(acc_full, (unsigned)(done & 1));
          tc_fence_after();
          if (dbg & 1) {
            tc_fence_before();
            __syncwarp();
            if (lane == 0) mbar_arrive_cluster(acc_empty, 0);
            continue;
          }
          const double sc = rb < NB ? sigma[rb * TM + (tid & 127)] * tau : 0.0;
          epilogue_row_block8(tmem, tid, warp, lane, sc, red + (done & 1) * (4 * TN),
                             rb < NB ? partial + ((long long)tile * NB + rb) * TN : nullptr, [&] { mbar_arrive_cluster(acc_empty, 0); });
        }
    }
  }
  tc_fence_before();
  __syncthreads();
  cluster_sync_all();
  if (warp == 8) asm volatile("tcgen05.dealloc.cta_group::2.sync.aligned.b32 %0, %1;\n" ::"r"(tmem), "n"(512) : "memory");
}

__global__ void __launch_bounds__(128)
posterior_i8_finish_kernel(const double* __restrict__ partial, const double* __restrict__ meanP, int NB, int Np,
                           const double* __restrict__ cand, long long rows, int d, const double* __restrict__ Xt,
                           const double* __restrict__ par, int kernel, double sf2, double mconst, double mean_scale,
                           long long cols_pad, double* __restrict__ mean, double* __restrict__ var) {
  const long long c = (long long)blockIdx.x * blockDim.x + threadIdx.x;
  if (c >= cols_pad) return;
  const double* p = partial + (c / TN) * NB * TN + c % TN;
  double run2 = 0.0, run1 = 0.0;
  for (int rb = 0; rb < NB; ++rb) run2 += p[(long long)rb * TN];
  const double* q = meanP + (c / TN) * (Np / 64) * 64 + c % TN;
  for (int kb = 0; kb < Np / 64; ++kb) run1 += q[(long long)kb * 64];
  double r2 = 0.0;
  if (c < rows)
    for (int j = 0; j < d; ++j) {
      const double t = (cand[c * d + j] - Xt[(long long)j * Np]) * par[j];
      r2 = fma(t, t, r2);
    }
  const bool nan_row = (r2 != r2) || (kernel == B7_KERNEL_MATERN52 && isinf(r2));
  const double poison = nan_row ? __longlong_as_double(0x7ff8000000000000LL) : 0.0;
  const double vv = sf2 - run2;
  var[c] = (vv > 0.0 ? vv : (vv != vv ? vv : 0.0)) + poison;
  mean[c] = (nan_row ? 0.0 : fma(run1, mean_scale, mconst)) + poison;
}

bool g_attr_i8[16] = {false};

}

size_t b7_i8_facs_stride(int Np) {
  const long long P = (Np / TM + 1) / 2;
  return (size_t)(4 * P * (P + 1)) * A_STAGE;
}

int b7_i8_slice_factor(b7_ctx* ctx, const double* fac, int Np, int8_t* facS, double* sigma, int s0, int count) {
  const int NBp = (Np / TM + 1) / 2 * 2;
  slice_factor_kernel<<<dim3(NBp, count), SLICE_THREADS, 0, ctx->stream>>>(fac, (long long)Np * Np, Np, facS, (long long)b7_i8_facs_stride(Np), sigma, s0);
  b7_count(ctx);
  B7_CUDA(cudaGetLastError());
  return 0;
}

template <int DT>
static int launch_cov_slices(b7_ctx* ctx, cudaStream_t st, int kernel, const double* A, int64_t rows, int64_t rows_pad, int d,
                             const double* Xt, int N, int Np, const double* par, double inv_tau, const double* alpha, int8_t* ksS,
                             double* meanP) {
  dim3 grid((unsigned)(rows_pad / TN), Np / 64);
  const bool se = kernel == B7_KERNEL_ARDSE;
  if (ctx->post_pair) {
    if (se) cov_slices_kernel<DT, B7_KERNEL_ARDSE, true><<<grid, 128, 0, st>>>(A, rows, d, Xt, N, Np, par, inv_tau, alpha, ksS, meanP);
    else cov_slices_kernel<DT, B7_KERNEL_MATERN52, true><<<grid, 128, 0, st>>>(A, rows, d, Xt, N, Np, par, inv_tau, alpha, ksS, meanP);
  } else {
    if (se) cov_slices_kernel<DT, B7_KERNEL_ARDSE, false><<<grid, 128, 0, st>>>(A, rows, d, Xt, N, Np, par, inv_tau, alpha, ksS, meanP);
    else cov_slices_kernel<DT, B7_KERNEL_MATERN52, false><<<grid, 128, 0, st>>>(A, rows, d, Xt, N, Np, par, inv_tau, alpha, ksS, meanP);
  }
  b7_count(ctx);
  B7_CUDA(cudaGetLastError());
  return 0;
}

int b7_i8_cov_slices(b7_ctx* ctx, cudaStream_t st, int kernel, const double* A, int64_t rows, int64_t rows_pad, int d, const double* Xt,
                     int N, int Np, const double* par, double tau, const double* alpha, int8_t* ksS, double* meanP) {
  if (rows_pad <= 0) return 0;
  const double inv_tau = 1.0 / tau;
#define B7_COV_SLICES(DT) return launch_cov_slices<DT>(ctx, st, kernel, A, rows, rows_pad, d, Xt, N, Np, par, inv_tau, alpha, ksS, meanP)
  if (d <= 2) B7_COV_SLICES(2);
  if (d <= 4) B7_COV_SLICES(4);
  if (d <= 6) B7_COV_SLICES(6);
  if (d <= 8) B7_COV_SLICES(8);
  if (d <= 12) B7_COV_SLICES(12);
  if (d <= 16) B7_COV_SLICES(16);
  if (d <= 20) B7_COV_SLICES(20);
  if (d <= 24) B7_COV_SLICES(24);
  if (d <= 32) B7_COV_SLICES(32);
  B7_COV_SLICES(40);
#undef B7_COV_SLICES
}

size_t b7_i8_partial_bytes(int Np, int64_t cols_pad) {
  return (size_t)(cols_pad / TN) * ((size_t)(Np / TM) * TN + (size_t)(Np / 64) * 64) * sizeof(double);
}
double* b7_i8_mean_partials(double* partial, int Np, int64_t cols_pad) { return partial + (size_t)(cols_pad / TN) * (Np / TM) * TN; }

int b7_launch_posterior_i8(b7_ctx* ctx, const int8_t* facS, const double* sigma, int Np, const int8_t* ksS, const double* cand,
                           int64_t rows, int d, const double* Xt, const double* par, int kernel, int64_t cols_pad, double tau,
                           double sf2, double mconst, double* partial, double* mean, double* var) {
  if (!g_attr_i8[ctx->device & 15]) {
    B7_CUDA(cudaFuncSetAttribute(posterior_i8_kernel, cudaFuncAttributeMaxDynamicSharedMemorySize, I8_SMEM));
    B7_CUDA(cudaFuncSetAttribute(posterior_i8_pair_kernel, cudaFuncAttributeMaxDynamicSharedMemorySize, P_SMEM));
    g_attr_i8[ctx->device & 15] = true;
  }
  if (cols_pad <= 0) return 0;
  const int NB = Np / TM;
  static const int group_env = getenv("B7_POST_GROUP") ? atoi(getenv("B7_POST_GROUP")) : 0;
  const int n_tiles = (int)(cols_pad / TN), group = group_env > 0 ? group_env : 16;
  if (ctx->post_pair) {
    const int P = (NB + 1) / 2, n_items = n_tiles * ((P + 1) / 2), n_pairs = ctx->sm_count / 2;
    static const int dbg_env = getenv("B7_POST_DBG") ? atoi(getenv("B7_POST_DBG")) : 0;
    posterior_i8_pair_kernel<<<2 * (n_items < n_pairs ? n_items : n_pairs), P_THREADS, P_SMEM, ctx->stream>>>(facS, sigma, Np, NB, ksS, tau, group,
                                                                                                              n_tiles, partial, dbg_env);
  } else {
    static const int chunk_env = getenv("B7_POST_CHUNK") ? atoi(getenv("B7_POST_CHUNK")) : 0;
    const int chunk = chunk_env > 0 ? (chunk_env < NB ? chunk_env : NB) : (NB < 2 ? NB : 2);
    const int cpt = (NB + chunk - 1) / chunk;
    const int n_items = n_tiles * ((cpt + 1) / 2);
    posterior_i8_kernel<<<n_items < ctx->sm_count ? n_items : ctx->sm_count, I8_THREADS, I8_SMEM, ctx->stream>>>(facS, sigma, Np, NB, ksS, tau, chunk,
                                                                                                                group, n_tiles, partial);
  }
  posterior_i8_finish_kernel<<<(unsigned)((cols_pad + 127) / 128), 128, 0, ctx->stream>>>(partial, b7_i8_mean_partials(partial, Np, cols_pad), NB, Np,
                                                                                         cand, rows, d, Xt, par, kernel, sf2, mconst,
                                                                                         tau * 5.5511151231257827e-17, cols_pad, mean, var);
  b7_count(ctx, 2);
  B7_CUDA(cudaGetLastError());
  return 0;
}
```

bot7_b200/csrc/potrf.cu:

```cuda
#include <stdio.h>
#include <stdlib.h>
#include <string.h>

#include <vector>

#include "b7_internal.h"
#include "gemm_tile.cuh"

using namespace b7g;

namespace {

constexpr int NBK = B7_NB;
constexpr int DIAG_THREADS = 512;
constexpr int DIAG_WARPS = DIAG_THREADS / 32;
constexpr int DLD = 132;
constexpr int SB = 16;
constexpr int DSLD = 20;
constexpr int TLD = 68;
constexpr int DIAG_SMEM = (NBK * DLD + 8 * SB * DSLD + 64 * TLD + 4 * NBK) * 8;

template <bool NN>
__device__ __forceinline__ void frag_mac(double& c0, double& c1, const double* __restrict__ A, int lda,
                                         const double* __restrict__ B, int ldb, int k_begin, int k_end, double sign, int lane) {
  const int r = lane >> 2, c = lane & 3;
#pragma unroll 2
  for (int k = k_begin; k < k_end; k += 4) {
    const double a = sign * A[r * lda + k + c];
    const double b = NN ? B[(k + c) * ldb + r] : B[r * ldb + k + c];
    dmma884(c0, c1, a, b);
  }
}

#ifdef B7_DIAG_STAMPS
__device__ long long b7_diag_stamps[128];
#define DIAG_STAMP(i) do { if (threadIdx.x == 0 && blockIdx.x == 0) b7_diag_stamps[i] = clock64(); } while (0)
#else
#define DIAG_STAMP(i) do { } while (0)
#endif

__device__ __forceinline__ void pdl_wait() { asm volatile("griddepcontrol.wait;" ::: "memory"); }
__device__ __forceinline__ void pdl_trigger() { asm volatile("griddepcontrol.launch_dependents;" ::: "memory"); }

constexpr int BAR_S1 = 1, BAR_U = 2, BAR_S2 = 3;
constexpr int UPD_THREADS = (DIAG_WARPS - DIAG_WARPS / 4) * 32;
__device__ __forceinline__ void nbar_sync(int id, int n) { asm volatile("bar.sync %0, %1;" ::"r"(id), "r"(n) : "memory"); }
__device__ __forceinline__ void nbar_arrive(int id, int n) { asm volatile("bar.arrive %0, %1;" ::"r"(id), "r"(n) : "memory"); }
__device__ __forceinline__ double rsq_seed(double x) {
  double y;
  asm("rsqrt.approx.ftz.f64 %0, %1;" : "=d"(y) : "d"(x));
  return y;
}

__device__ __forceinline__ void fence_cta() { asm volatile("fence.acq_rel.cta;" ::: "memory"); }

__device__ __forceinline__ void diag_subpanel(double* M, const double* DSp, int i0, int j0, int g, int lane) {
  const int r = lane >> 2, c = lane & 3;
  double* Arow = M + (i0 + 8 * g) * DLD + j0;
  double a4[4];
#pragma unroll
  for (int k4 = 0; k4 < 4; ++k4) a4[k4] = Arow[r * DLD + 4 * k4 + c];
  double c00 = 0, c01 = 0, c10 = 0, c11 = 0;
#pragma unroll
  for (int k4 = 0; k4 < 4; ++k4) {
    dmma884(c00, c01, a4[k4], DSp[r * DSLD + 4 * k4 + c]);
    dmma884(c10, c11, a4[k4], DSp[(8 + r) * DSLD + 4 * k4 + c]);
  }
  __syncwarp();
  *reinterpret_cast<double2*>(Arow + r * DLD + 2 * c) = make_double2(c00, c01);
  *reinterpret_cast<double2*>(Arow + r * DLD + 8 + 2 * c) = make_double2(c10, c11);
}

__device__ __forceinline__ void diag_subpanel_pair(double* M, const double* DSp, int i0, int j0, int lane) {
  const int r = lane >> 2, c = lane & 3;
  double* Arow = M + i0 * DLD + j0;
  double a0[4], a1[4], b0[4], b1[4];
#pragma unroll
  for (int k4 = 0; k4 < 4; ++k4) {
    a0[k4] = Arow[r * DLD + 4 * k4 + c];
    a1[k4] = Arow[(8 + r) * DLD + 4 * k4 + c];
    b0[k4] = DSp[r * DSLD + 4 * k4 + c];
    b1[k4] = DSp[(8 + r) * DSLD + 4 * k4 + c];
  }
  double c00 = 0, c01 = 0, c10 = 0, c11 = 0, e00 = 0, e01 = 0, e10 = 0, e11 = 0;
#pragma unroll
  for (int k4 = 0; k4 < 4; ++k4) {
    dmma884(c00, c01, a0[k4], b0[k4]);
    dmma884(c10, c11, a0[k4], b1[k4]);
    dmma884(e00, e01, a1[k4], b0[k4]);
    dmma884(e10, e11, a1[k4], b1[k4]);
  }
  __syncwarp();
  *reinterpret_cast<double2*>(Arow + r * DLD + 2 * c) = make_double2(c00, c01);
  *reinterpret_cast<double2*>(Arow + r * DLD + 8 + 2 * c) = make_double2(c10, c11);
  *reinterpret_cast<double2*>(Arow + (8 + r) * DLD + 2 * c) = make_double2(e00, e01);
  *reinterpret_cast<double2*>(Arow + (8 + r) * DLD + 8 + 2 * c) = make_double2(e10, e11);
}

__device__ __forceinline__ void diag_trail_next_piece(double* M, int i0, int j0, int lane) {
  const int r = lane >> 2, c = lane & 3;
  const double* L0 = M + i0 * DLD + j0;
  double a0[4], a1[4];
#pragma unroll
  for (int k4 = 0; k4 < 4; ++k4) {
    a0[k4] = L0[r * DLD + 4 * k4 + c];
    a1[k4] = L0[(8 + r) * DLD + 4 * k4 + c];
  }
  double2* p00 = reinterpret_cast<double2*>(M + (i0 + r) * DLD + i0 + 2 * c);
  double2* p10 = reinterpret_cast<double2*>(M + (i0 + 8 + r) * DLD + i0 + 2 * c);
  double2* p11 = reinterpret_cast<double2*>(M + (i0 + 8 + r) * DLD + i0 + 8 + 2 * c);
  double2 v00 = *p00, v10 = *p10, v11 = *p11;
#pragma unroll
  for (int k4 = 0; k4 < 4; ++k4) {
    dmma884(v00.x, v00.y, -a0[k4], a0[k4]);
    dmma884(v10.x, v10.y, -a1[k4], a0[k4]);
    dmma884(v11.x, v11.y, -a1[k4], a1[k4]);
  }
  *p00 = v00; *p10 = v10; *p11 = v11;
}

__device__ __forceinline__ void diag_trail_frag(double* M, int i0, int j0, int gi, int gk, int lane) {
  const int r = lane >> 2, c = lane & 3;
  double2* cp = reinterpret_cast<double2*>(M + (i0 + 8 * gi + r) * DLD + i0 + 8 * gk + 2 * c);
  double2 cv = *cp;
  frag_mac<false>(cv.x, cv.y, M + (i0 + 8 * gi) * DLD + j0, DLD, M + (i0 + 8 * gk) * DLD + j0, DLD, 0, SB, -1.0, lane);
  *cp = cv;
}

__device__ __forceinline__ void diag_store_tile(double* __restrict__ blk, const double* M, int kt, int t, int nthreads) {
  for (int u = t; u < NBK * 8; u += nthreads) {
    const int i = (u >> 1) & 127, k0 = kt * TILE_K + (u >> 8) * 4 + (u & 1) * 2;
    const double2 v = *reinterpret_cast<const double2*>(M + i * DLD + k0);
    *reinterpret_cast<double2*>(blk + kt * TILE_DOUBLES + u * 2) = make_double2(k0 <= i ? v.x : 0.0, k0 + 1 <= i ? v.y : 0.0);
  }
}

__global__ void __launch_bounds__(DIAG_THREADS, 1)
diag_kernel(double* __restrict__ fac, long long fac_stride, int Np, int j, double* __restrict__ dinv, long long dinv_stride,
            double* __restrict__ beta, double* __restrict__ logdet, int* __restrict__ info, int s0) {
  extern __shared__ __align__(16) double sm[];
  double* M = sm;
  double* DS = M + NBK * DLD;
  double* T = DS + 8 * SB * DSLD;
  double* pivs = T + 64 * TLD;
  double* invs = pivs + NBK;
  double* rj = invs + NBK;
  double* lg = rj + NBK;
  __shared__ int s_info;
  const int s = s0 + blockIdx.x, tid = threadIdx.x, warp = tid >> 5, lane = tid & 31;
  const int r = lane >> 2, c = lane & 3;
  DIAG_STAMP(0);
  pdl_wait();
  double* blk = fac + (long long)s * fac_stride + tile_off(Np / TILE_K, j, j * (NBK / TILE_K));
#pragma unroll 8
  for (int u = tid; u < NBK * NBK / 2; u += DIAG_THREADS) {
    const int i = (u >> 1) & 127, k0 = (u >> 10) * TILE_K + ((u >> 8) & 3) * 4 + (u & 1) * 2;
    double2 v = make_double2(0.0, 0.0);
    if (k0 <= i) v = *reinterpret_cast<const double2*>(blk + 2 * u);
    *reinterpret_cast<double2*>(M + i * DLD + k0) = make_double2(v.x, k0 + 1 <= i ? v.y : 0.0);
  }
  if (tid < NBK) rj[tid] = beta[(long long)s * Np + j * NBK + tid];
  if (tid == 0) s_info = 0;
  __syncthreads();
  DIAG_STAMP(1);

  if (warp == 0) {
    const bool is_row = lane < SB;
    const int li = lane & (SB - 1);
    int my_info = 0;
    for (int p = 0; p < NBK / SB; ++p) {
      const int j0 = p * SB, i0 = j0 + SB;
      double a[SB], d[SB];
#pragma unroll
      for (int k = 0; k < SB; ++k) {
        a[k] = is_row ? M[(j0 + li) * DLD + j0 + k] : (k == li ? 1.0 : 0.0);
        d[k] = M[(j0 + k) * DLD + j0 + k];
      }
      double mypiv = 1.0, myinv = 1.0;
#pragma unroll
      for (int q = 0; q < SB; ++q) {
        const double piv = d[q];
        const double y = rsq_seed(piv);
        const double ay = a[q] * y, t = y * y;
        const double e = fma(-piv, t, 1.0);
        const double u = fma(e, 0.375, 0.5);
        const double my = fma(u, ay * e, ay);
        const double inv = fma(u, y * e, y);
        if (lane == q) { mypiv = piv; myinv = inv; }
#pragma unroll
        for (int k = 0; k < SB; ++k) {
          if (k > q) {
            const double lk = __shfl_sync(0xffffffffu, my, k);
            a[k] = fma(-my, lk, a[k]);
            d[k] = fma(-lk, lk, d[k]);
          }
        }
        a[q] = my;
      }
      const unsigned bad = __ballot_sync(0xffffffffu, is_row && (!(mypiv > 0.0) || !(myinv > 0.0) || myinv > 1.79e308));
      if (bad != 0u && my_info == 0) my_info = j * NBK + j0 + __ffs((int)bad);
      if (is_row) {
#pragma unroll
        for (int k = 0; k < SB; k += 2)
          *reinterpret_cast<double2*>(M + (j0 + lane) * DLD + j0 + k) = make_double2(k <= lane ? a[k] : 0.0, k + 1 <= lane ? a[k + 1] : 0.0);
        pivs[j0 + lane] = mypiv;
        invs[j0 + lane] = myinv;
      } else {
#pragma unroll
        for (int i = 0; i < SB; ++i) DS[(p * SB + i) * DSLD + li] = a[i];
      }
      __syncwarp();
      DIAG_STAMP(2 + 3 * p);
      if (p < NBK / SB - 1) {
        if (p >= 1) nbar_sync(BAR_S2, 32 + UPD_THREADS);
        DIAG_STAMP(3 + 3 * p);
        diag_subpanel_pair(M, DS + p * SB * DSLD, i0, j0, lane);
        if (p < NBK / SB - 2) {
          fence_cta();
          nbar_arrive(BAR_S1, 32 + UPD_THREADS);
        }
        __syncwarp();
        diag_trail_next_piece(M, i0, j0, lane);
        __syncwarp();
        DIAG_STAMP(4 + 3 * p);
      }
    }
    if (lane == 0) s_info = my_info;
  } else if ((warp & 3) != 0) {
    const int uw = warp - 1 - (warp >> 2), ut = uw * 32 + lane;
    constexpr int UW = UPD_THREADS / 32;
    for (int p = 0; p < NBK / SB - 2; ++p) {
      const int j0 = p * SB, i0 = j0 + SB, G = (NBK - i0) / 8;
      nbar_sync(BAR_S1, 32 + UPD_THREADS);
      if (ut < SB) lg[j0 + ut] = log(pivs[j0 + ut] * invs[j0 + ut]);
      for (int g = 2 + uw; g < G; g += UW) diag_subpanel(M, DS + p * SB * DSLD, i0, j0, g, lane);
      nbar_sync(BAR_U, UPD_THREADS);
      const int n_frag = G * (G + 1) / 2;
      int gi = 2, rem = uw;
      for (int f = 3 + uw; f < n_frag; f += UW) {
        while (rem > gi) { rem -= gi + 1; ++gi; }
        diag_trail_frag(M, i0, j0, gi, rem, lane);
        rem += UW;
      }
      fence_cta();
      nbar_arrive(BAR_S2, 32 + UPD_THREADS);
      diag_store_tile(blk, M, p, ut, UPD_THREADS);
    }
  }
  __syncthreads();
  DIAG_STAMP(26);
  diag_store_tile(blk, M, NBK / SB - 2, tid, DIAG_THREADS);
  diag_store_tile(blk, M, NBK / SB - 1, tid, DIAG_THREADS);
  if (tid >= NBK - 2 * SB && tid < NBK) lg[tid] = log(pivs[tid] * invs[tid]);
  __syncthreads();
  for (int e = tid; e < NBK * SB; e += DIAG_THREADS) {
    const int i = e >> 4, k = e & 15;
    M[i * DLD + (i & ~15) + k] = DS[i * DSLD + k];
  }
  __syncthreads();
  DIAG_STAMP(27);
  for (int h = SB; h < NBK; h <<= 1) {
    const int fpr = h / 8, wpp = DIAG_WARPS / (NBK / (2 * h));
    const int t = warp / wpp, wl = warp % wpp, base = 2 * h * t;
    const int half = fpr / 2, lo = wl % half, ypw = wpp / half;
    for (int fi = wl / half; fi < fpr; fi += ypw)
      for (int m = 0; m < 2; ++m) {
        const int fn = m == 0 ? lo : fpr - 1 - lo;
        double c0 = 0.0, c1 = 0.0;
        frag_mac<true>(c0, c1, M + (base + h + 8 * fi) * DLD + base, DLD, M + base * DLD + base + 8 * fn, DLD, 8 * fn, h, 1.0, lane);
        *reinterpret_cast<double2*>(T + (t * h + 8 * fi + r) * TLD + 8 * fn + 2 * c) = make_double2(c0, c1);
      }
    __syncthreads();
    DIAG_STAMP(h == 16 ? 28 : h == 32 ? 30 : 32);
    for (int fn = wl / half; fn < fpr; fn += ypw)
      for (int m = 0; m < 2; ++m) {
        const int fi = m == 0 ? lo : fpr - 1 - lo;
        double c0 = 0.0, c1 = 0.0;
        frag_mac<true>(c0, c1, M + (base + h + 8 * fi) * DLD + base + h, DLD, T + (t * h) * TLD + 8 * fn, TLD, 0, 8 * fi + 8, -1.0, lane);
        *reinterpret_cast<double2*>(M + (base + h + 8 * fi + r) * DLD + base + 8 * fn + 2 * c) = make_double2(c0, c1);
      }
    __syncthreads();
    DIAG_STAMP(h == 16 ? 29 : h == 32 ? 31 : 33);
  }
  pdl_trigger();
  {
    const int row = tid >> 2, part = tid & 3;
    double xv = 0.0;
    for (int k = part; k <= row; k += 4) xv = fma(M[row * DLD + k], rj[k], xv);
    xv += __shfl_xor_sync(0xffffffffu, xv, 1);
    xv += __shfl_xor_sync(0xffffffffu, xv, 2);
    if (part == 0) beta[(long long)s * Np + j * NBK + row] = xv;
  }
  DIAG_STAMP(34);
  double* di = dinv + (long long)s * dinv_stride + (long long)j * NBK * NBK;
#pragma unroll 4
  for (int u = tid; u < NBK * NBK / 2; u += DIAG_THREADS) {
    const int i = (u >> 1) & 127, k0 = (u >> 10) * TILE_K + ((u >> 8) & 3) * 4 + (u & 1) * 2;
    if (k0 <= i) {
      const double2 v = *reinterpret_cast<const double2*>(M + i * DLD + k0);
      *reinterpret_cast<double2*>(di + 2 * u) = make_double2(v.x, k0 + 1 <= i ? v.y : 0.0);
    }
  }
  if (tid == 0) {
    double ld_acc = 0.0;
    for (int q = 0; q < NBK; ++q) ld_acc += lg[q];
    logdet[s] = (j == 0 ? 0.0 : logdet[s]) + ld_acc;
    const int my_info = s_info;
    if (j == 0) info[s] = my_info;
    else if (info[s] == 0 && my_info != 0) info[s] = my_info;
  }
  DIAG_STAMP(35);
}

__global__ void dinv_transpose_kernel(const double* __restrict__ dinv, double* __restrict__ dinvT, long long dinv_stride, int s0) {
  const long long off = (long long)(s0 + blockIdx.y) * dinv_stride + (long long)blockIdx.x * NBK * NBK;
  const double* di = dinv + off;
  double* dt = dinvT + off;
  for (int e = threadIdx.x; e < NBK * NBK; e += blockDim.x) {
    const int kk = e & 3, i = (e >> 2) & 127, k = (e >> 11) * TILE_K + ((e >> 9) & 3) * 4 + kk;
    dt[e] = (k >= i) ? di[elem_off(k, i)] : 0.0;
  }
}

__global__ void __launch_bounds__(THREADS, 1)
panel_kernel(double* __restrict__ fac, long long fac_stride, int Np, int j, const double* __restrict__ dinv,
             long long dinv_stride, double* __restrict__ beta, int s0) {
  extern __shared__ __align__(128) double smem[];
  const int s = s0 + blockIdx.z, it = j + 1 + blockIdx.x, KPB = NBK / TILE_K;
  double* tile = fac + (long long)s * fac_stride + tile_off(Np / TILE_K, it, j * KPB);
  const double* B = dinv + (long long)s * dinv_stride + (long long)j * NBK * NBK;
  Ring ring; ring.init(smem);
  Acc acc; acc.zero();
  mainloop_bulk(ring, tile, B, KPB, acc);
  const int tid = threadIdx.x, warp = tid >> 5, lane = tid & 31, wm = warp >> 2, wn = warp & 3;
  const double* xj = beta + (long long)s * Np + j * NBK;
  double* red = smem;
#pragma unroll
  for (int i = 0; i < 8; ++i) {
    const int row = frag_row(wm, i, lane);
    double part = 0.0;
#pragma unroll
    for (int jj = 0; jj < 4; ++jj) {
      const int col = frag_col(wn, jj, lane);
      *reinterpret_cast<double2*>(tile + elem_off(row, col)) = make_double2(acc.c[i][jj][0], acc.c[i][jj][1]);
      part += acc.c[i][jj][0] * xj[col] + acc.c[i][jj][1] * xj[col + 1];
    }
    part += __shfl_xor_sync(0xffffffffu, part, 1);
    part += __shfl_xor_sync(0xffffffffu, part, 2);
    if ((lane & 3) == 0) red[row * 4 + wn] = part;
  }
  __syncthreads();
  if (tid < NBK) {
    double sum = ((red[tid * 4 + 0] + red[tid * 4 + 1]) + red[tid * 4 + 2]) + red[tid * 4 + 3];
    beta[(long long)s * Np + it * NBK + tid] -= sum;
  }
}

__global__ void __launch_bounds__(THREADS, 1)
trail_kernel(double* __restrict__ fac, long long fac_stride, int Np, int kb0, int kb1, int it0, int nt0, int s0) {
  extern __shared__ __align__(128) double smem[];
  const int it = it0 + blockIdx.x, nt = nt0 + blockIdx.y;
  if (nt > it) return;
  const int s = s0 + blockIdx.z, KPB = NBK / TILE_K, KTA = Np / TILE_K;
  double* base = fac + (long long)s * fac_stride;
  const double* A = base + tile_off(KTA, it, kb0 * KPB);
  const double* B = base + tile_off(KTA, nt, kb0 * KPB);
  double* C = base + tile_off(KTA, it, nt * KPB);
  Ring ring; ring.init(smem);
  const int warp = threadIdx.x >> 5, lane = threadIdx.x & 31, wm = warp >> 2, wn = warp & 3;
  if (threadIdx.x == 0)
    for (int p = 0; p < 2 && p < (kb1 - kb0) * KPB; ++p) ring.produce(A + (long long)p * TILE_DOUBLES, B + (long long)p * TILE_DOUBLES);
  Acc acc;
#pragma unroll
  for (int i = 0; i < 8; ++i)
#pragma unroll
    for (int jj = 0; jj < 4; ++jj) {
      const double2 v = *reinterpret_cast<const double2*>(C + elem_off(frag_row(wm, i, lane), frag_col(wn, jj, lane)));
      acc.c[i][jj][0] = -v.x;
      acc.c[i][jj][1] = -v.y;
    }
  mainloop_bulk(ring, A, B, (kb1 - kb0) * KPB, acc, 2);
#pragma unroll
  for (int i = 0; i < 8; ++i)
#pragma unroll
    for (int jj = 0; jj < 4; ++jj)
      *reinterpret_cast<double2*>(C + elem_off(frag_row(wm, i, lane), frag_col(wn, jj, lane))) =
          make_double2(-acc.c[i][jj][0], -acc.c[i][jj][1]);
}

constexpr int SL_ROWS = 16, SL_STAGES = 6, SL_AHEAD = 5, SL_THREADS = (SL_ROWS / 16) * 128, SL_SPLIT = NBK / SL_ROWS;
constexpr int SL_A_DOUBLES = SL_ROWS * TILE_K;
constexpr int SL_STAGE_DOUBLES = TILE_DOUBLES + SL_A_DOUBLES;
constexpr int SL_SMEM = SL_STAGES * SL_STAGE_DOUBLES * 8 + 256;

struct SliceAcc { double c[2][4][2]; };

struct SliceRing {
  double* smem;
  uint64_t *full, *empty;
  int issued, consumed;
  __device__ __forceinline__ void init(double* base) {
    smem = base;
    full = reinterpret_cast<uint64_t*>(base + SL_STAGES * SL_STAGE_DOUBLES);
    empty = full + SL_STAGES;
    issued = consumed = 0;
    if (threadIdx.x == 0) {
      for (int st = 0; st < SL_STAGES; ++st) { mbar_init(full + st, 1); mbar_init(empty + st, SL_THREADS / 32); }
      mbar_fence_init();
    }
    __syncthreads();
  }
  __device__ __forceinline__ void produce(const double* a_tile, const double* b_tile, int r0) {
    const int slot = issued % SL_STAGES;
    if (issued >= SL_STAGES) mbar_wait(empty + slot, (unsigned)(((issued / SL_STAGES) - 1) & 1));
    double* st = smem + slot * SL_STAGE_DOUBLES;
    mbar_arrive_expect_tx(full + slot, SL_STAGE_DOUBLES * 8);
    bulk_g2s(st, b_tile, TILE_DOUBLES * 8, full + slot);
#pragma unroll
    for (int g4 = 0; g4 < KG; ++g4)
      bulk_g2s(st + TILE_DOUBLES + g4 * (SL_ROWS * 4), a_tile + g4 * (BM * 4) + r0 * 4, SL_ROWS * 4 * 8, full + slot);
    ++issued;
  }
};

__device__ __forceinline__ void slice_mainloop(SliceRing& ring, const double* __restrict__ gA, const double* __restrict__ gB, int KT, int r0,
                                               SliceAcc& acc) {
  const int tid = threadIdx.x, warp = tid >> 5, lane = tid & 31, wm = warp >> 2, wn = warp & 3;
  int p = 0;
  if (tid == 0)
    for (; p < SL_AHEAD && p < KT; ++p) ring.produce(gA + (long long)p * TILE_DOUBLES, gB + (long long)p * TILE_DOUBLES, r0);
  for (int kt = 0; kt < KT; ++kt) {
    if (tid == 0 && p < KT) { ring.produce(gA + (long long)p * TILE_DOUBLES, gB + (long long)p * TILE_DOUBLES, r0); ++p; }
    const int slot = ring.consumed % SL_STAGES;
    mbar_wait(ring.full + slot, (unsigned)((ring.consumed / SL_STAGES) & 1));
    const double* sB = ring.smem + slot * SL_STAGE_DOUBLES;
    const double* sA = sB + TILE_DOUBLES;
#pragma unroll
    for (int g4 = 0; g4 < KG; ++g4) {
      double a[2], b[4];
      const double* pa = sA + g4 * (SL_ROWS * 4) + (16 * wm) * 4 + lane;
      const double* pb = sB + g4 * (BN * 4) + (32 * wn) * 4 + lane;
#pragma unroll
      for (int i = 0; i < 2; ++i) a[i] = pa[i * 32];
#pragma unroll
      for (int jj = 0; jj < 4; ++jj) b[jj] = pb[jj * 32];
#pragma unroll
      for (int i = 0; i < 2; ++i)
#pragma unroll
        for (int jj = 0; jj < 4; ++jj) dmma884(acc.c[i][jj][0], acc.c[i][jj][1], a[i], b[jj]);
    }
    __syncwarp();
    if (lane == 0) mbar_arrive(ring.empty + slot);
    ++ring.consumed;
  }
  __syncthreads();
}

__device__ __forceinline__ int sl_row(int wm, int i, int lane) { return 16 * wm + 8 * i + (lane >> 2); }

__global__ void __launch_bounds__(SL_THREADS, 2)
panel_slice_kernel(double* __restrict__ fac, long long fac_stride, int Np, int j, const double* __restrict__ dinv,
                   long long dinv_stride, double* __restrict__ beta, int s0) {
  extern __shared__ __align__(128) double smem[];
  const int s = s0 + blockIdx.z, it = j + 1 + blockIdx.y, r0 = blockIdx.x * SL_ROWS, KPB = NBK / TILE_K;
  double* tile = fac + (long long)s * fac_stride + tile_off(Np / TILE_K, it, j * KPB);
  const double* B = dinv + (long long)s * dinv_stride + (long long)j * NBK * NBK;
  SliceRing ring; ring.init(smem);
  SliceAcc acc;
#pragma unroll
  for (int i = 0; i < 2; ++i)
#pragma unroll
    for (int jj = 0; jj < 4; ++jj) acc.c[i][jj][0] = acc.c[i][jj][1] = 0.0;
  pdl_trigger();
  pdl_wait();
  slice_mainloop(ring, tile, B, KPB, r0, acc);
  const int tid = threadIdx.x, warp = tid >> 5, lane = tid & 31, wm = warp >> 2, wn = warp & 3;
  const double* xj = beta + (long long)s * Np + j * NBK;
  double* red = smem;
#pragma unroll
  for (int i = 0; i < 2; ++i) {
    const int row = sl_row(wm, i, lane);
    double part = 0.0;
#pragma unroll
    for (int jj = 0; jj < 4; ++jj) {
      const int col = frag_col(wn, jj, lane);
      *reinterpret_cast<double2*>(tile + elem_off(r0 + row, col)) = make_double2(acc.c[i][jj][0], acc.c[i][jj][1]);
      part += acc.c[i][jj][0] * xj[col] + acc.c[i][jj][1] * xj[col + 1];
    }
    part += __shfl_xor_sync(0xffffffffu, part, 1);
    part += __shfl_xor_sync(0xffffffffu, part, 2);
    if ((lane & 3) == 0) red[row * 4 + wn] = part;
  }
  __syncthreads();
  if (tid < SL_ROWS) {
    double sum = ((red[tid * 4 + 0] + red[tid * 4 + 1]) + red[tid * 4 + 2]) + red[tid * 4 + 3];
    beta[(long long)s * Np + it * NBK + r0 + tid] -= sum;
  }
}

__global__ void __launch_bounds__(SL_THREADS, 2)
trail_slice_kernel(double* __restrict__ fac, long long fac_stride, int Np, int kb0, int kb1, int it0, int nt0, int s0) {
  extern __shared__ __align__(128) double smem[];
  const int it = it0 + (int)(blockIdx.x / SL_SPLIT), nt = nt0 + blockIdx.y, r0 = (int)(blockIdx.x % SL_SPLIT) * SL_ROWS;
  pdl_trigger();
  if (nt > it) { pdl_wait(); return; }
  const int s = s0 + blockIdx.z, KPB = NBK / TILE_K, KTA = Np / TILE_K;
  double* base = fac + (long long)s * fac_stride;
  const double* A = base + tile_off(KTA, it, kb0 * KPB);
  const double* B = base + tile_off(KTA, nt, kb0 * KPB);
  double* C = base + tile_off(KTA, it, nt * KPB);
  SliceRing ring; ring.init(smem);
  pdl_wait();
  const int warp = threadIdx.x >> 5, lane = threadIdx.x & 31, wm = warp >> 2, wn = warp & 3;
  SliceAcc acc;
#pragma unroll
  for (int i = 0; i < 2; ++i)
#pragma unroll
    for (int jj = 0; jj < 4; ++jj) {
      const double2 v = *reinterpret_cast<const double2*>(C + elem_off(r0 + sl_row(wm, i, lane), frag_col(wn, jj, lane)));
      acc.c[i][jj][0] = -v.x;
      acc.c[i][jj][1] = -v.y;
    }
  slice_mainloop(ring, A, B, (kb1 - kb0) * KPB, r0, acc);
#pragma unroll
  for (int i = 0; i < 2; ++i)
#pragma unroll
    for (int jj = 0; jj < 4; ++jj)
      *reinterpret_cast<double2*>(C + elem_off(r0 + sl_row(wm, i, lane), frag_col(wn, jj, lane))) =
          make_double2(-acc.c[i][jj][0], -acc.c[i][jj][1]);
}

__global__ void place_diag_kernel(double* __restrict__ fac, long long fac_stride, int Np, const double* __restrict__ dinv,
                                  long long dinv_stride, int s0) {
  const int s = s0 + blockIdx.y, j = blockIdx.x;
  double* blk = fac + (long long)s * fac_stride + tile_off(Np / TILE_K, j, j * (NBK / TILE_K));
  const double* di = dinv + (long long)s * dinv_stride + (long long)j * NBK * NBK;
  for (int e = threadIdx.x; e < NBK * NBK; e += blockDim.x) blk[e] = di[e];
}

__global__ void __launch_bounds__(THREADS, 1)
inv_step1_kernel(const double* __restrict__ fac, long long fac_stride, int Np, int j, const double* __restrict__ dinvT,
                 long long dinv_stride, double* __restrict__ tt, long long tt_stride, int s0) {
  extern __shared__ __align__(128) double smem[];
  const int s = s0 + blockIdx.z, it = j + 1 + blockIdx.x, KPB = NBK / TILE_K;
  const double* A = fac + (long long)s * fac_stride + tile_off(Np / TILE_K, it, j * KPB);
  const double* B = dinvT + (long long)s * dinv_stride + (long long)j * NBK * NBK;
  Ring ring; ring.init(smem);
  Acc acc; acc.zero();
  mainloop_bulk(ring, A, B, KPB, acc);
  const int warp = threadIdx.x >> 5, lane = threadIdx.x & 31, wm = warp >> 2, wn = warp & 3;
  double* T = tt + (long long)s * tt_stride;
#pragma unroll
  for (int i = 0; i < 8; ++i)
#pragma unroll
    for (int jj = 0; jj < 4; ++jj) {
      const int k = it * NBK + frag_row(wm, i, lane), col = frag_col(wn, jj, lane);
      T[elem_off(col, k)] = acc.c[i][jj][0];
      T[elem_off(col + 1, k)] = acc.c[i][jj][1];
    }
}

__global__ void __launch_bounds__(THREADS, 1)
inv_step2_kernel(double* __restrict__ fac, long long fac_stride, int Np, int j, const double* __restrict__ tt,
                 long long tt_stride, int s0) {
  extern __shared__ __align__(128) double smem[];
  const int n_it = gridDim.x, it = j + n_it - (int)blockIdx.x, KPB = NBK / TILE_K, KTA = Np / TILE_K;
  const int s = s0 + blockIdx.z;
  double* base = fac + (long long)s * fac_stride;
  const double* A = base + tile_off(KTA, it, (j + 1) * KPB);
  const double* B = tt + (long long)s * tt_stride + (long long)(j + 1) * KPB * TILE_DOUBLES;
  double* C = base + tile_off(KTA, it, j * KPB);
  Ring ring; ring.init(smem);
  Acc acc; acc.zero();
  mainloop_bulk(ring, A, B, (it - j) * KPB, acc);
  const int warp = threadIdx.x >> 5, lane = threadIdx.x & 31, wm = warp >> 2, wn = warp & 3;
#pragma unroll
  for (int i = 0; i < 8; ++i)
#pragma unroll
    for (int jj = 0; jj < 4; ++jj)
      *reinterpret_cast<double2*>(C + elem_off(frag_row(wm, i, lane), frag_col(wn, jj, lane))) =
          make_double2(-acc.c[i][jj][0], -acc.c[i][jj][1]);
}

__global__ void untile_kernel(const double* __restrict__ facT, double* __restrict__ out, int Np, int N) {
  const int row = blockIdx.x;
  const double* src = facT + tile_off(Np / TILE_K, row >> 7, 0);
  for (int k = threadIdx.x; k < N; k += blockDim.x) out[(long long)row * N + k] = src[elem_off(row & 127, k)];
}

bool g_attr_done[16] = {false};
int set_attrs(int device) {
  if (g_attr_done[device & 15]) return 0;
  auto set = [](const void* fn, int smem) -> cudaError_t {
    cudaError_t e = cudaFuncSetAttribute(fn, cudaFuncAttributeMaxDynamicSharedMemorySize, smem);
    if (e != cudaSuccess) return e;
    return cudaFuncSetAttribute(fn, cudaFuncAttributePreferredSharedMemoryCarveout, cudaSharedmemCarveoutMaxShared);
  };
  B7_CUDA(set((const void*)diag_kernel, DIAG_SMEM));
  B7_CUDA(set((const void*)panel_kernel, RING_SMEM));
  B7_CUDA(set((const void*)trail_kernel, RING_SMEM));
  B7_CUDA(set((const void*)panel_slice_kernel, SL_SMEM));
  B7_CUDA(set((const void*)trail_slice_kernel, SL_SMEM));
  B7_CUDA(set((const void*)inv_step1_kernel, RING_SMEM));
  B7_CUDA(set((const void*)inv_step2_kernel, RING_SMEM));
  g_attr_done[device & 15] = true;
  return 0;
}

constexpr int ALPHA_THREADS = 1024;

template <bool FROM_INVERSE>
__global__ void __launch_bounds__(ALPHA_THREADS, 1)
alpha_kernel(const double* __restrict__ fac, long long fac_stride, int Np, const double* __restrict__ dinvT, long long dinv_stride,
             const double* __restrict__ beta, double* __restrict__ alpha, int s0) {
  extern __shared__ __align__(16) double sm[];
  double* r = sm;
  double* xa = sm + Np;
  const int s = s0 + blockIdx.x, tid = threadIdx.x, warp = tid >> 5, lane = tid & 31, NB = Np / NBK;
  const double* F = fac + (long long)s * fac_stride;
  for (int e = tid; e < Np; e += ALPHA_THREADS) r[e] = FROM_INVERSE ? 0.0 : beta[(long long)s * Np + e];
  __syncthreads();
  for (int step = 0; step < NB; ++step) {
    const int ib = FROM_INVERSE ? step : NB - 1 - step;
    if (tid < NBK) {
      if (FROM_INVERSE) {
        xa[tid] = beta[(long long)s * Np + ib * NBK + tid];
      } else {
        const double* dt = dinvT + (long long)s * dinv_stride + (long long)ib * NBK * NBK;
        double sum = 0.0;
#pragma unroll 4
        for (int q4 = 0; q4 < NBK / 4; ++q4) {
          const double4 m = *reinterpret_cast<const double4*>(dt + (q4 >> 2) * TILE_DOUBLES + (q4 & 3) * (BM * 4) + tid * 4);
          const double* rr = r + ib * NBK + 4 * q4;
          sum = fma(m.x, rr[0], sum); sum = fma(m.y, rr[1], sum); sum = fma(m.z, rr[2], sum); sum = fma(m.w, rr[3], sum);
        }
        xa[tid] = sum;
        alpha[(long long)s * Np + ib * NBK + tid] = sum;
      }
    }
    __syncthreads();
    const double* rowblk = F + tile_off(Np / TILE_K, ib, 0);
    const int n_kg = (FROM_INVERSE ? ib + 1 : ib) * (NBK / 4);
    for (int kg = warp; kg < n_kg; kg += ALPHA_THREADS / 32) {
      const double* p = rowblk + (long long)kg * (BM * 4);
      double4 v[4];
#pragma unroll
      for (int i = 0; i < 4; ++i) v[i] = *reinterpret_cast<const double4*>(p + (lane + 32 * i) * 4);
      double a0 = 0.0, a1 = 0.0, a2 = 0.0, a3 = 0.0;
#pragma unroll
      for (int i = 0; i < 4; ++i) {
        const double x = xa[lane + 32 * i];
        a0 = fma(v[i].x, x, a0); a1 = fma(v[i].y, x, a1); a2 = fma(v[i].z, x, a2); a3 = fma(v[i].w, x, a3);
      }
#pragma unroll
      for (int o = 16; o > 0; o >>= 1) {
        a0 += __shfl_xor_sync(0xffffffffu, a0, o); a1 += __shfl_xor_sync(0xffffffffu, a1, o);
        a2 += __shfl_xor_sync(0xffffffffu, a2, o); a3 += __shfl_xor_sync(0xffffffffu, a3, o);
      }
      if (lane == 0) {
        double* out = r + kg * 4;
        if (FROM_INVERSE) { out[0] += a0; out[1] += a1; out[2] += a2; out[3] += a3; }
        else { out[0] -= a0; out[1] -= a1; out[2] -= a2; out[3] -= a3; }
      }
    }
    __syncthreads();
  }
  if (FROM_INVERSE)
    for (int e = tid; e < Np; e += ALPHA_THREADS) alpha[(long long)s * Np + e] = r[e];
}

struct PotrfTrace {
  bool on = false;
  cudaStream_t st = nullptr;
  std::vector<cudaEvent_t> ev;
  std::vector<const char*> tag;
  void mark(const char* name) {
    if (!on) return;
    cudaEvent_t e;
    cudaEventCreate(&e);
    cudaEventRecord(e, st);
    ev.push_back(e);
    tag.push_back(name);
  }
  void dump() {
    if (!on) return;
    cudaStreamSynchronize(st);
    const char* names[] = {"diag", "panel", "trail", "slice", "near", "wait_far", "transpose"};
    double sum[7] = {0, 0, 0, 0, 0, 0, 0};
    int cnt[7] = {0, 0, 0, 0, 0, 0, 0};
    for (size_t i = 1; i < ev.size(); ++i) {
      float ms = 0.f;
      cudaEventElapsedTime(&ms, ev[i - 1], ev[i]);
      for (int k = 0; k < 7; ++k)
        if (strcmp(tag[i], names[k]) == 0) { sum[k] += ms; ++cnt[k]; }
      if (getenv("B7_POTRF_TRACE") && atoi(getenv("B7_POTRF_TRACE")) > 1) fprintf(stderr, "  %-10s %8.1f us\n", tag[i], ms * 1e3);
    }
    float total = 0.f;
    if (ev.size() > 1) cudaEventElapsedTime(&total, ev.front(), ev.back());
    fprintf(stderr, "potrf trace: total %.1f us;", total * 1e3);
    for (int k = 0; k < 7; ++k)
      if (cnt[k]) fprintf(stderr, " %s %d x %.1f us;", names[k], cnt[k], sum[k] * 1e3 / cnt[k]);
    fprintf(stderr, "\n");
    for (cudaEvent_t e : ev) cudaEventDestroy(e);
  }
};

int potrf_latency_enqueue(b7_gp* gp, int s0, int count, int W, bool allow_trace);

int potrf_latency(b7_gp* gp, int s0, int count, int W) {
  b7_ctx* ctx = gp->ctx;
  static const int graph_env = getenv("B7_POTRF_GRAPH") ? atoi(getenv("B7_POTRF_GRAPH")) : -1;
  const bool graph_ok = graph_env >= 0 ? graph_env != 0 : gp->NB <= 16;
  if (!graph_ok || getenv("B7_POTRF_TRACE")) return potrf_latency_enqueue(gp, s0, count, W, true);
  if (gp->potrf_graph && gp->potrf_graph_s0 == s0 && gp->potrf_graph_count == count) {
    B7_CUDA(cudaGraphLaunch(gp->potrf_graph, ctx->stream));
    b7_count(ctx, gp->potrf_graph_launches);
    return 0;
  }
  if (gp->potrf_calls_s0 == s0 && gp->potrf_calls_count == count) ++gp->potrf_calls;
  else { gp->potrf_calls_s0 = s0; gp->potrf_calls_count = count; gp->potrf_calls = 1; }
  if (gp->potrf_calls < 2) return potrf_latency_enqueue(gp, s0, count, W, false);
  if (gp->potrf_graph) { cudaGraphExecDestroy(gp->potrf_graph); gp->potrf_graph = nullptr; }
  const int64_t before = ctx->launches;
  cudaGraph_t graph = nullptr;
  B7_CUDA(cudaStreamBeginCapture(ctx->stream, cudaStreamCaptureModeThreadLocal));
  const int rc = potrf_latency_enqueue(gp, s0, count, W, false);
  const cudaError_t e = cudaStreamEndCapture(ctx->stream, &graph);
  if (rc != 0 || e != cudaSuccess || graph == nullptr) {
    if (getenv("B7_DEBUG")) fprintf(stderr, "potrf graph: capture failed (rc %d, %s)\n", rc, cudaGetErrorString(e));
    if (graph) cudaGraphDestroy(graph);
    cudaGetLastError();
    ctx->launches = before;
    gp->potrf_calls = -(1 << 30);
    return potrf_latency_enqueue(gp, s0, count, W, false);
  }
  const cudaError_t ei = cudaGraphInstantiate(&gp->potrf_graph, graph, 0);
  cudaGraphDestroy(graph);
  if (ei != cudaSuccess) {
    if (getenv("B7_DEBUG")) fprintf(stderr, "potrf graph: instantiation failed (%s)\n", cudaGetErrorString(ei));
    gp->potrf_graph = nullptr;
    cudaGetLastError();
    ctx->launches = before;
    gp->potrf_calls = -(1 << 30);
    return potrf_latency_enqueue(gp, s0, count, W, false);
  }
  gp->potrf_graph_s0 = s0;
  gp->potrf_graph_count = count;
  gp->potrf_graph_launches = (int)(ctx->launches - before);
  if (getenv("B7_DEBUG")) fprintf(stderr, "potrf graph: %d kernel nodes captured\n", gp->potrf_graph_launches);
  B7_CUDA(cudaGraphLaunch(gp->potrf_graph, ctx->stream));
  return 0;
}

template <typename... KArgs, typename... Args>
cudaError_t launch_pdl(void (*kernel)(KArgs...), dim3 grid, dim3 block, size_t smem, cudaStream_t st, bool pdl, Args... args) {
  cudaLaunchConfig_t cfg = {};
  cfg.gridDim = grid;
  cfg.blockDim = block;
  cfg.dynamicSmemBytes = smem;
  cfg.stream = st;
  int prio = 0;
  cudaStreamGetPriority(st, &prio);
  cudaLaunchAttribute attr[2];
  attr[0].id = cudaLaunchAttributePriority;
  attr[0].val.priority = prio;
  attr[1].id = cudaLaunchAttributeProgrammaticStreamSerialization;
  attr[1].val.programmaticStreamSerializationAllowed = 1;
  cfg.attrs = attr;
  cfg.numAttrs = pdl ? 2 : 1;
  return cudaLaunchKernelEx(&cfg, kernel, KArgs(args)...);
}

int potrf_latency_enqueue(b7_gp* gp, int s0, int count, int W, bool allow_trace) {
  b7_ctx* ctx = gp->ctx;
  static const bool pdl = !(getenv("B7_POTRF_PDL") && atoi(getenv("B7_POTRF_PDL")) == 0);
  const int Np = gp->Np, NB = gp->NB, SPT = NBK / SL_ROWS;
  const long long fs = (long long)Np * Np, ds = (long long)NB * NBK * NBK;
  cudaStream_t sa = ctx->stream, sb = ctx->stream2, sc = ctx->stream3;
  bool far_pending = false, side_pending = false, near1_pending = false;
  PotrfTrace trace;
  trace.on = allow_trace && getenv("B7_POTRF_TRACE") != nullptr;
  trace.st = sa;
  trace.mark("start");
  auto trail = [&](cudaStream_t st, int kb0, int kb1, int it0, int n_it, int nt0, int n_nt) {
    launch_pdl(trail_slice_kernel, dim3(n_it * SPT, n_nt, count), dim3(SL_THREADS), SL_SMEM, st, pdl && st == sa, gp->fac, fs, Np, kb0, kb1, it0, nt0, s0);
    b7_count(ctx);
  };
  for (int J = 0; J < NB; J += W) {
    const int Jend = J + W < NB ? J + W : NB;
    for (int j = J; j < Jend; ++j) {
      launch_pdl(diag_kernel, dim3(count), dim3(DIAG_THREADS), DIAG_SMEM, sa, pdl && j > 0, gp->fac, fs, Np, j, gp->dinv, ds, gp->beta, gp->logdet,
                 gp->info, s0);
      b7_count(ctx);
      trace.mark("diag");
      const int rem = NB - 1 - j;
      if (rem > 0) {
        launch_pdl(panel_slice_kernel, dim3(SPT, rem, count), dim3(SL_THREADS), SL_SMEM, sa, pdl, gp->fac, fs, Np, j, (const double*)gp->dinv, ds, gp->beta, s0);
        b7_count(ctx);
        trace.mark("panel");
      }
      if (j + 1 < Jend) {
        if (near1_pending) { B7_CUDA(cudaStreamWaitEvent(sa, ctx->evS1, 0)); near1_pending = false; }
        if (side_pending && j > J) { B7_CUDA(cudaStreamWaitEvent(sa, ctx->evS, 0)); side_pending = false; }
        trail(sa, j, j + 1, j + 1, rem, j + 1, 1);
        trace.mark("trail");
        if (j + 2 < Jend) {
          B7_CUDA(cudaEventRecord(ctx->evA, sa));
          B7_CUDA(cudaStreamWaitEvent(sc, ctx->evA, 0));
          trail(sc, j, j + 1, j + 2, rem - 1, j + 2, Jend - 2 - j);
          B7_CUDA(cudaEventRecord(ctx->evS, sc));
          side_pending = true;
        }
      }
    }
    if (Jend >= NB) break;
    const int near_end = Jend + W < NB ? Jend + W : NB;
    if (side_pending) { B7_CUDA(cudaStreamWaitEvent(sa, ctx->evS, 0)); side_pending = false; }
    if (far_pending) B7_CUDA(cudaStreamWaitEvent(sa, ctx->evB, 0));
    trace.mark("wait_far");
    trail(sa, J, Jend, Jend, NB - Jend, Jend, 1);
    trace.mark("near");
    B7_CUDA(cudaEventRecord(ctx->evA, sa));
    if (near_end - Jend > 1) {
      B7_CUDA(cudaStreamWaitEvent(sc, ctx->evA, 0));
      trail(sc, J, Jend, Jend + 1, NB - Jend - 1, Jend + 1, 1);
      B7_CUDA(cudaEventRecord(ctx->evS1, sc));
      near1_pending = true;
      if (near_end - Jend > 2) {
        trail(sc, J, Jend, Jend + 2, NB - Jend - 2, Jend + 2, near_end - Jend - 2);
        B7_CUDA(cudaEventRecord(ctx->evS, sc));
        side_pending = true;
      }
    }
    if (near_end < NB) {
      B7_CUDA(cudaStreamWaitEvent(sb, ctx->evA, 0));
      trail(sb, J, Jend, near_end, NB - near_end, near_end, NB - near_end);
      B7_CUDA(cudaEventRecord(ctx->evB, sb));
      far_pending = true;
    }
  }
  if (far_pending) B7_CUDA(cudaStreamWaitEvent(sa, ctx->evB, 0));
  if (side_pending) B7_CUDA(cudaStreamWaitEvent(sa, ctx->evS, 0));
  if (near1_pending) B7_CUDA(cudaStreamWaitEvent(sa, ctx->evS1, 0));
  trace.mark("wait_far");
  dinv_transpose_kernel<<<dim3(NB, count), 512, 0, sa>>>(gp->dinv, gp->dinvT, ds, s0);
  b7_count(ctx);
  trace.mark("transpose");
  trace.dump();
  B7_CUDA(cudaGetLastError());
  return 0;
}

}

int b7_launch_potrf(b7_gp* gp, int s0, int count) {
  b7_ctx* ctx = gp->ctx;
  B7_CHECK(set_attrs(ctx->device));
  const int Np = gp->Np, NB = gp->NB;
  const long long fs = (long long)Np * Np, ds = (long long)NB * NBK * NBK;
  static const int W_env = getenv("B7_POTRF_W") ? atoi(getenv("B7_POTRF_W")) : 0;
  const int W = W_env > 0 ? W_env : 4;
  static const int slice_env = getenv("B7_POTRF_SLICE") ? atoi(getenv("B7_POTRF_SLICE")) : -1;
  const bool small_batch = (long long)gp->S * NB * NB <= 2048;
  if (slice_env >= 0 ? slice_env != 0 : (count <= 2 || small_batch)) return potrf_latency(gp, s0, count, W);
  cudaStream_t sa = ctx->stream, sb = ctx->stream2;
  bool far_pending = false;
  PotrfTrace trace;
  trace.on = getenv("B7_POTRF_TRACE") != nullptr;
  trace.st = sa;
  trace.mark("start");
  const int batch = gp->S;
  const bool i8 = ctx->use_i8 && ctx->potrf_i8 && batch >= 4 && (long long)batch * NB * NB >= 4096 && NB > W && Np <= B7_I8_MAX_NP;
  int8_t* pS[2][2] = {{nullptr, nullptr}, {nullptr, nullptr}};
  double* pSig[2] = {nullptr, nullptr};
  const size_t p_stride = i8 ? b7_i8_panel_bytes(Np, W) : 0;
  if (i8)
    for (int b = 0; b < 2; ++b) {
      B7_CHECK(b7_pool_alloc(ctx, (void**)&pS[b][0], p_stride * count));
      B7_CHECK(b7_pool_alloc(ctx, (void**)&pS[b][1], p_stride * count));
      B7_CHECK(b7_pool_alloc(ctx, (void**)&pSig[b], sizeof(double) * (size_t)Np * count));
    }
  int set = 0;
  for (int J = 0; J < NB; J += W) {
    const int Jend = J + W < NB ? J + W : NB;
    for (int j = J; j < Jend; ++j) {
      diag_kernel<<<count, DIAG_THREADS, DIAG_SMEM, sa>>>(gp->fac, fs, Np, j, gp->dinv, ds, gp->beta, gp->logdet, gp->info, s0);
      b7_count(ctx);
      trace.mark("diag");
      const int rem = NB - 1 - j;
      if (rem > 0) {
        panel_kernel<<<dim3(rem, 1, count), THREADS, RING_SMEM, sa>>>(gp->fac, fs, Np, j, gp->dinv, ds, gp->beta, s0);
        b7_count(ctx);
        trace.mark("panel");
      }
      if (Jend - 1 - j > 0) {
        trail_kernel<<<dim3(rem, Jend - 1 - j, count), THREADS, RING_SMEM, sa>>>(gp->fac, fs, Np, j, j + 1, j + 1, j + 1, s0);
        b7_count(ctx);
        trace.mark("trail");
      }
    }
    if (Jend >= NB) break;
    const int near_end = Jend + W < NB ? Jend + W : NB;
    if (i8) B7_CHECK(b7_i8_panel_slice(ctx, sa, gp->fac, Np, J, Jend, Jend, pS[set][0], pS[set][1], p_stride, pSig[set], s0, count));
    if (far_pending) B7_CUDA(cudaStreamWaitEvent(sa, ctx->evB, 0));
    trace.mark("wait_far");
    if (i8) {
      B7_CHECK(b7_i8_trail(ctx, sa, gp->fac, Np, pS[set][0], pS[set][1], p_stride, pSig[set], J, Jend, Jend, Jend, NB - Jend, Jend,
                           near_end - Jend, s0, count));
    } else {
      trail_kernel<<<dim3(NB - Jend, near_end - Jend, count), THREADS, RING_SMEM, sa>>>(gp->fac, fs, Np, J, Jend, Jend, Jend, s0);
      b7_count(ctx);
    }
    trace.mark("near");
    if (near_end < NB) {
      B7_CUDA(cudaEventRecord(ctx->evA, sa));
      B7_CUDA(cudaStreamWaitEvent(sb, ctx->evA, 0));
      if (i8) {
        B7_CHECK(b7_i8_trail(ctx, sb, gp->fac, Np, pS[set][0], pS[set][1], p_stride, pSig[set], J, Jend, Jend, near_end, NB - near_end,
                             near_end, NB - near_end, s0, count));
      } else {
        trail_kernel<<<dim3(NB - near_end, NB - near_end, count), THREADS, RING_SMEM, sb>>>(gp->fac, fs, Np, J, Jend, near_end, near_end, s0);
        b7_count(ctx);
      }
      B7_CUDA(cudaEventRecord(ctx->evB, sb));
      far_pending = true;
    }
    set ^= 1;
  }
  if (far_pending) B7_CUDA(cudaStreamWaitEvent(sa, ctx->evB, 0));
  trace.mark("wait_far");
  dinv_transpose_kernel<<<dim3(NB, count), 512, 0, sa>>>(gp->dinv, gp->dinvT, ds, s0);
  b7_count(ctx);
  trace.mark("transpose");
  trace.dump();
  if (i8)
    for (int b = 0; b < 2; ++b) {
      b7_pool_free(ctx, pS[b][0]);
      b7_pool_free(ctx, pS[b][1]);
      b7_pool_free(ctx, pSig[b]);
    }
  B7_CUDA(cudaGetLastError());
  return 0;
}

int b7_launch_alpha(b7_gp* gp, int s0, int count, bool from_inverse) {
  b7_ctx* ctx = gp->ctx;
  const int Np = gp->Np;
  const size_t smem = (size_t)(Np + NBK) * sizeof(double);
  if (smem > 200 * 1024) { b7_set_error("alpha: %d observations exceed the shared-memory sweep", Np); return B7_ERR_ARG; }
  static bool attr[16][2] = {{false}};
  if (!attr[ctx->device & 15][from_inverse]) {
    if (from_inverse) B7_CUDA(cudaFuncSetAttribute(alpha_kernel<true>, cudaFuncAttributeMaxDynamicSharedMemorySize, 200 * 1024));
    else B7_CUDA(cudaFuncSetAttribute(alpha_kernel<false>, cudaFuncAttributeMaxDynamicSharedMemorySize, 200 * 1024));
    attr[ctx->device & 15][from_inverse] = true;
  }
  const long long fs = (long long)Np * Np, ds = (long long)gp->NB * NBK * NBK;
  if (from_inverse) alpha_kernel<true><<<count, ALPHA_THREADS, smem, ctx->stream>>>(gp->fac, fs, Np, gp->dinvT, ds, gp->beta, gp->alpha, s0);
  else alpha_kernel<false><<<count, ALPHA_THREADS, smem, ctx->stream>>>(gp->fac, fs, Np, gp->dinvT, ds, gp->beta, gp->alpha, s0);
  b7_count(ctx);
  B7_CUDA(cudaGetLastError());
  return 0;
}

int b7_launch_untile(b7_ctx* ctx, const double* facT, double* out, int Np, int N) {
  untile_kernel<<<N, 256, 0, ctx->stream>>>(facT, out, Np, N);
  b7_count(ctx);
  B7_CUDA(cudaGetLastError());
  return 0;
}

int b7_launch_trtri(b7_gp* gp, int s0, int count) {
  b7_ctx* ctx = gp->ctx;
  B7_CHECK(set_attrs(ctx->device));
  const int Np = gp->Np, NB = gp->NB;
  const long long fs = (long long)Np * Np, ds = (long long)NB * NBK * NBK, ts = (long long)NBK * Np;
  place_diag_kernel<<<dim3(NB, count), 256, 0, ctx->stream>>>(gp->fac, fs, Np, gp->dinv, ds, s0);
  b7_count(ctx);
  if (ctx->use_i8 && ctx->trtri_i8 && Np <= B7_I8_MAX_NP) return b7_launch_trtri_i8(gp, s0, count);
  for (int j = NB - 2; j >= 0; --j) {
    const int rem = NB - 1 - j;
    inv_step1_kernel<<<dim3(rem, 1, count), THREADS, RING_SMEM, ctx->stream>>>(gp->fac, fs, Np, j, gp->dinvT, ds, gp->tt, ts, s0);
    inv_step2_kernel<<<dim3(rem, 1, count), THREADS, RING_SMEM, ctx->stream>>>(gp->fac, fs, Np, j, gp->tt, ts, s0);
    b7_count(ctx, 2);
  }
  B7_CUDA(cudaGetLastError());
  return 0;
}
```

Before: 187,200.

## Chain K* slicing into posterior pass via PDL co-residency on one stream

Replaces the two-stream event ping-pong between the K* covariance-slice kernel and the int8 posterior kernel with a single-stream chain. A persistent, atomic-work-queue variant of cov_slices (64 threads) is launched with programmatic dependent launch so it runs alongside the posterior kernel, which now triggers dependents early. The posterior finish kernel is split out so the next K* (including the first hyper of the next panel) is enqueued between the main and finish passes. This aims to remove cross-stream event overhead and idle gaps, at the cost of register and shared-memory occupancy checks, a work-counter allocation, and more complex buffer ping-pong indexing.

```diff
diff --git a/bot7_b200/csrc/api.cu b/bot7_b200/csrc/api.cu
--- a/bot7_b200/csrc/api.cu
+++ b/bot7_b200/csrc/api.cu
@@ -215,10 +215,6 @@
   B7_CUDA(cudaStreamCreateWithPriority(&ctx->stream3, cudaStreamNonBlocking, (prio_hi + prio_lo) / 2));
   B7_CUDA(cudaEventCreateWithFlags(&ctx->evS, cudaEventDisableTiming));
   B7_CUDA(cudaEventCreateWithFlags(&ctx->evS1, cudaEventDisableTiming));
-  for (int i = 0; i < 2; ++i) {
-    B7_CUDA(cudaEventCreateWithFlags(&ctx->evK[i], cudaEventDisableTiming));
-    B7_CUDA(cudaEventCreateWithFlags(&ctx->evP[i], cudaEventDisableTiming));
-  }
   { const char* e = getenv("B7_KSTAR_OVERLAP"); ctx->kstar_overlap = !(e && e[0] == '0'); }
   cudaMemPoolProps props = {};
   props.allocType = cudaMemAllocationTypePinned;
@@ -264,7 +260,6 @@
   cudaStreamDestroy(ctx->stream3);
   cudaEventDestroy(ctx->evA);
   cudaEventDestroy(ctx->evB);
-  for (int i = 0; i < 2; ++i) { cudaEventDestroy(ctx->evK[i]); cudaEventDestroy(ctx->evP[i]); }
   cudaStreamDestroy(ctx->stream2);
   cudaEventDestroy(ctx->ev0);
   cudaEventDestroy(ctx->ev1);
@@ -752,14 +747,15 @@
     B7_CHECK(grow(ctx, &ctx->i8_partial, &ctx->i8_partial_bytes, b7_i8_partial_bytes(gp->Np, rp64)));
     {
       StageTimer t(ctx, ST_KSTAR);
-      B7_CHECK(b7_i8_cov_slices(ctx, ctx->stream, gp->kernel, A, rows, rp64, gp->d, gp->Xt, gp->N, gp->Np, gp->par + (size_t)s * kParStride, tau,
+      B7_CHECK(b7_i8_cov_slices(ctx, gp->kernel, A, rows, rp64, gp->d, gp->Xt, gp->N, gp->Np, gp->par + (size_t)s * kParStride, tau,
                                 gp->alpha + (size_t)s * gp->Np, ksS, b7_i8_mean_partials(ctx->i8_partial, gp->Np, rp64)));
       t.stop(1);
     }
     StageTimer t(ctx, ST_POSTERIOR);
-    B7_CHECK(b7_launch_posterior_i8(ctx, gp->facS + (size_t)s * b7_i8_facs_stride(gp->Np), gp->sigma + (size_t)s * gp->Np, gp->Np, ksS, A, rows,
-                                    gp->d, gp->Xt, gp->par + (size_t)s * kParStride, gp->kernel, rp64, tau, p[B7_MAX_DIMS], p[B7_MAX_DIMS + 2],
-                                    ctx->i8_partial, mean, var));
+    B7_CHECK(b7_launch_posterior_i8(ctx, gp->facS + (size_t)s * b7_i8_facs_stride(gp->Np), gp->sigma + (size_t)s * gp->Np, gp->Np, ksS, rp64, tau,
+                                    ctx->i8_partial));
+    B7_CHECK(b7_launch_posterior_i8_finish(ctx, gp->Np, A, rows, gp->d, gp->Xt, gp->par + (size_t)s * kParStride, gp->kernel, rp64, tau,
+                                           p[B7_MAX_DIMS], p[B7_MAX_DIMS + 2], ctx->i8_partial, mean, var));
     t.stop(1);
     return 0;
   }
@@ -778,44 +774,62 @@
   return 0;
 }
 
-static int posterior_panel_draws_i8(b7_gp* gp, const double* A, int64_t rows, double* dm, double* dv, int64_t ld) {
+struct KstarChain {
+  b7_ctx* ctx = nullptr;
+  size_t ks_bytes = 0, part_bytes = 0;
+  int* work = nullptr;
+  int g = 0;
+  bool primed = false;
+  explicit KstarChain(b7_ctx* c) : ctx(c) {}
+  ~KstarChain() { dev_free(ctx, work); }
+};
+
+static int kstar_chain_begin(b7_gp* gp, KstarChain& ch, int64_t max_rows, int64_t n_panels) {
+  b7_ctx* ctx = gp->ctx;
+  const int64_t rp64 = (max_rows + 63) / 64 * 64;
+  ch.ks_bytes = ((size_t)rp64 * gp->Np * B7_I8_SLICES + 255) / 256 * 256;
+  ch.part_bytes = (b7_i8_partial_bytes(gp->Np, rp64) + 255) / 256 * 256;
+  B7_CHECK(grow(ctx, &ctx->ks, &ctx->ks_bytes, 2 * ch.ks_bytes));
+  B7_CHECK(grow(ctx, &ctx->i8_partial, &ctx->i8_partial_bytes, 2 * ch.part_bytes));
+  for (int s = 0; s < gp->S; ++s)
+    if (!gp->sliced[s]) B7_CHECK(gp_slice(gp, s, 1));
+  const size_t n_work = (size_t)n_panels * gp->S + 1;
+  B7_CHECK(dev_alloc(ctx, &ch.work, n_work));
+  B7_CUDA(cudaMemsetAsync(ch.work, 0, n_work * sizeof(int), ctx->stream));
+  return 0;
+}
+
+static int posterior_panel_draws_i8(b7_gp* gp, KstarChain& ch, const double* A, int64_t rows, double* dm, double* dv, int64_t ld,
+                                    const double* A_next, int64_t rows_next) {
   b7_ctx* ctx = gp->ctx;
   const int S = gp->S;
   const int64_t rp64 = (rows + 63) / 64 * 64;
-  const size_t ks_bytes = ((size_t)rp64 * gp->Np * B7_I8_SLICES + 255) / 256 * 256;
-  const size_t part_bytes = (b7_i8_partial_bytes(gp->Np, rp64) + 255) / 256 * 256;
-  B7_CHECK(grow(ctx, &ctx->ks, &ctx->ks_bytes, 2 * ks_bytes));
-  B7_CHECK(grow(ctx, &ctx->i8_partial, &ctx->i8_partial_bytes, 2 * part_bytes));
-  for (int s = 0; s < S; ++s)
-    if (!gp->sliced[s]) B7_CHECK(gp_slice(gp, s, 1));
   auto tau_of = [&](int s) {
     int e = 0;
     frexp(gp->par_host[(size_t)s * kParStride + B7_MAX_DIMS], &e);
     return ldexp(1.0, e);
   };
-  auto ks_of = [&](int s) { return reinterpret_cast<int8_t*>(ctx->ks) + (size_t)(s & 1) * ks_bytes; };
-  auto part_of = [&](int s) { return reinterpret_cast<double*>(reinterpret_cast<char*>(ctx->i8_partial) + (size_t)(s & 1) * part_bytes); };
-  auto kstar = [&](int s) {
-    return b7_i8_cov_slices(ctx, ctx->stream2, gp->kernel, A, rows, rp64, gp->d, gp->Xt, gp->N, gp->Np, gp->par + (size_t)s * kParStride, tau_of(s),
-                            gp->alpha + (size_t)s * gp->Np, ks_of(s), b7_i8_mean_partials(part_of(s), gp->Np, rp64));
+  auto ks_of = [&](int g) { return reinterpret_cast<int8_t*>(ctx->ks) + (size_t)(g & 1) * ch.ks_bytes; };
+  auto part_of = [&](int g) { return reinterpret_cast<double*>(reinterpret_cast<char*>(ctx->i8_partial) + (size_t)(g & 1) * ch.part_bytes); };
+  auto kstar = [&](int g, int s, const double* X, int64_t n, int* work) {
+    const int64_t n64 = (n + 63) / 64 * 64;
+    return b7_i8_cov_slices(ctx, gp->kernel, X, n, n64, gp->d, gp->Xt, gp->N, gp->Np, gp->par + (size_t)s * kParStride, tau_of(s),
+                            gp->alpha + (size_t)s * gp->Np, ks_of(g), b7_i8_mean_partials(part_of(g), gp->Np, n64), work);
   };
-  B7_CUDA(cudaEventRecord(ctx->evA, ctx->stream));
-  B7_CUDA(cudaStreamWaitEvent(ctx->stream2, ctx->evA, 0));
-  B7_CHECK(kstar(0));
-  B7_CUDA(cudaEventRecord(ctx->evK[0], ctx->stream2));
+  const int g0 = ch.g;
+  if (!ch.primed) B7_CHECK(kstar(g0, 0, A, rows, nullptr));
   for (int s = 0; s < S; ++s) {
-    if (s + 1 < S) {
-      if (s >= 1) B7_CUDA(cudaStreamWaitEvent(ctx->stream2, ctx->evP[(s + 1) & 1], 0));
-      B7_CHECK(kstar(s + 1));
-      B7_CUDA(cudaEventRecord(ctx->evK[(s + 1) & 1], ctx->stream2));
-    }
-    B7_CUDA(cudaStreamWaitEvent(ctx->stream, ctx->evK[s & 1], 0));
+    const int g = g0 + s;
     const double* p = gp->par_host.data() + (size_t)s * kParStride;
-    B7_CHECK(b7_launch_posterior_i8(ctx, gp->facS + (size_t)s * b7_i8_facs_stride(gp->Np), gp->sigma + (size_t)s * gp->Np, gp->Np, ks_of(s), A, rows,
-                                    gp->d, gp->Xt, gp->par + (size_t)s * kParStride, gp->kernel, rp64, tau_of(s), p[B7_MAX_DIMS], p[B7_MAX_DIMS + 2],
-                                    part_of(s), dm + (size_t)s * ld, dv + (size_t)s * ld));
-    B7_CUDA(cudaEventRecord(ctx->evP[s & 1], ctx->stream));
-  }
+    B7_CHECK(b7_launch_posterior_i8(ctx, gp->facS + (size_t)s * b7_i8_facs_stride(gp->Np), gp->sigma + (size_t)s * gp->Np, gp->Np, ks_of(g),
+                                    rp64, tau_of(s), part_of(g)));
+    if (s + 1 < S) B7_CHECK(kstar(g + 1, s + 1, A, rows, ch.work + g + 1));
+    else if (A_next) B7_CHECK(kstar(g + 1, 0, A_next, rows_next, ch.work + g + 1));
+    B7_CHECK(b7_launch_posterior_i8_finish(ctx, gp->Np, A, rows, gp->d, gp->Xt, gp->par + (size_t)s * kParStride, gp->kernel, rp64, tau_of(s),
+                                           p[B7_MAX_DIMS], p[B7_MAX_DIMS + 2], part_of(g), dm + (size_t)s * ld, dv + (size_t)s * ld));
+  }
+  ch.g = g0 + S;
+  ch.primed = A_next != nullptr;
   return 0;
 }
 
@@ -904,11 +918,16 @@
   if (score_host) B7_CHECK(dev_alloc(ctx, &sb.p, (size_t)std::max<int64_t>(count, 1)));
   double* const score_dev = sb.p;
   int n_parts = 0, rc = 0;
+  const bool chain = i8_path(gp) && ctx->kstar_overlap && !ctx->profiling && S > 1 && all_sliced_or_sliceable(gp) &&
+                     b7_i8_kstar_chains(ctx, gp->kernel, gp->d);
+  KstarChain ch(ctx);
+  if (chain) B7_CHECK(kstar_chain_begin(gp, ch, std::min(P, count), n_panels));
   for (int64_t c0 = 0; c0 < count && rc == 0; c0 += P) {
     const int64_t n = std::min(P, count - c0), np = pad128(n);
     double* dm = ctx->moments; double* dv = ctx->moments + (size_t)S * np;
-    if (i8_path(gp) && ctx->kstar_overlap && !ctx->profiling && S > 1 && all_sliced_or_sliceable(gp))
-      rc = posterior_panel_draws_i8(gp, grid->X + (row0 + c0) * grid->d, n, dm, dv, np);
+    if (chain)
+      rc = posterior_panel_draws_i8(gp, ch, grid->X + (row0 + c0) * grid->d, n, dm, dv, np,
+                                    c0 + P < count ? grid->X + (row0 + c0 + P) * grid->d : nullptr, std::min(P, count - c0 - P));
     else
       for (int s = 0; s < S && rc == 0; ++s)
         rc = posterior_panel(gp, s, grid->X + (row0 + c0) * grid->d, n, dm + (size_t)s * np, dv + (size_t)s * np);
diff --git a/bot7_b200/csrc/b7_internal.h b/bot7_b200/csrc/b7_internal.h
--- a/bot7_b200/csrc/b7_internal.h
+++ b/bot7_b200/csrc/b7_internal.h
@@ -38,7 +38,6 @@
   cudaStream_t stream2 = nullptr;
   cudaStream_t stream3 = nullptr;
   cudaEvent_t evA = nullptr, evB = nullptr, evS = nullptr, evS1 = nullptr;
-  cudaEvent_t evK[2] = {nullptr, nullptr}, evP[2] = {nullptr, nullptr};
   bool kstar_overlap = true;
   cudaEvent_t ev0 = nullptr, ev1 = nullptr, tm0 = nullptr, tm1 = nullptr;
   double stage_ms[ST_COUNT] = {0};
@@ -154,6 +153,28 @@
   }
 };
 
+__device__ __forceinline__ void pdl_wait() { asm volatile("griddepcontrol.wait;" ::: "memory"); }
+__device__ __forceinline__ void pdl_trigger() { asm volatile("griddepcontrol.launch_dependents;" ::: "memory"); }
+
+template <typename... KArgs, typename... Args>
+cudaError_t launch_pdl(void (*kernel)(KArgs...), dim3 grid, dim3 block, size_t smem, cudaStream_t st, bool pdl, Args... args) {
+  cudaLaunchConfig_t cfg = {};
+  cfg.gridDim = grid;
+  cfg.blockDim = block;
+  cfg.dynamicSmemBytes = smem;
+  cfg.stream = st;
+  int prio = 0;
+  cudaStreamGetPriority(st, &prio);
+  cudaLaunchAttribute attr[2];
+  attr[0].id = cudaLaunchAttributePriority;
+  attr[0].val.priority = prio;
+  attr[1].id = cudaLaunchAttributeProgrammaticStreamSerialization;
+  attr[1].val.programmaticStreamSerializationAllowed = 1;
+  cfg.attrs = attr;
+  cfg.numAttrs = pdl ? 2 : 1;
+  return cudaLaunchKernelEx(&cfg, kernel, KArgs(args)...);
+}
+
 void b7_sobol_directions_host(int dims, uint32_t* out );
 int b7_launch_sobol(b7_ctx* ctx, int dims, int64_t first_seed, int64_t count, const double* mins_dev,
                     const double* maxes_dev, double* out_dev);
@@ -176,11 +197,14 @@
 #define B7_I8_MAX_NP 16384
 size_t b7_i8_facs_stride(int Np);
 int b7_i8_slice_factor(b7_ctx* ctx, const double* fac, int Np, int8_t* facS, double* sigma, int s0, int count);
-int b7_i8_cov_slices(b7_ctx* ctx, cudaStream_t st, int kernel, const double* A, int64_t rows, int64_t rows_pad, int d, const double* Xt,
-                     int N, int Np, const double* par, double tau, const double* alpha, int8_t* ksS, double* meanP);
-int b7_launch_posterior_i8(b7_ctx* ctx, const int8_t* facS, const double* sigma, int Np, const int8_t* ksS, const double* cand,
-                           int64_t rows, int d, const double* Xt, const double* par, int kernel, int64_t cols_pad, double tau,
-                           double sf2, double mconst, double* partial, double* mean, double* var);
+int b7_i8_cov_slices(b7_ctx* ctx, int kernel, const double* A, int64_t rows, int64_t rows_pad, int d, const double* Xt,
+                     int N, int Np, const double* par, double tau, const double* alpha, int8_t* ksS, double* meanP, int* work = nullptr);
+bool b7_i8_kstar_chains(b7_ctx* ctx, int kernel, int d);
+int b7_launch_posterior_i8(b7_ctx* ctx, const int8_t* facS, const double* sigma, int Np, const int8_t* ksS, int64_t cols_pad, double tau,
+                           double* partial);
+int b7_launch_posterior_i8_finish(b7_ctx* ctx, int Np, const double* cand, int64_t rows, int d, const double* Xt, const double* par,
+                                  int kernel, int64_t cols_pad, double tau, double sf2, double mconst, const double* partial, double* mean,
+                                  double* var);
 size_t b7_i8_partial_bytes(int Np, int64_t cols_pad);
 double* b7_i8_mean_partials(double* partial, int Np, int64_t cols_pad);
 int b7_launch_score(b7_ctx* ctx, int kind, const double* mean, const double* var, int S, int64_t M, int64_t ld,
diff --git a/bot7_b200/csrc/posterior_i8.cu b/bot7_b200/csrc/posterior_i8.cu
--- a/bot7_b200/csrc/posterior_i8.cu
+++ b/bot7_b200/csrc/posterior_i8.cu
@@ -1,5 +1,7 @@
 #include <math.h>
 #include <stdlib.h>
+
+#include <unordered_map>
 
 #include "b7_internal.h"
 #include "exp_neg.cuh"
@@ -29,6 +31,7 @@
 constexpr int P_STAGE = A_STAGE + B_HALF;
 constexpr int P_NSTAGE = 3;
 constexpr int P_SMEM = P_NSTAGE * P_STAGE + RED_BYTES + 1024;
+constexpr int KSTAR_CHAIN_THREADS = 64;
 constexpr int P_THREADS = 320;
 static_assert(P_STAGE % 1024 == 0 && P_SMEM <= 227 * 1024, "pair stage geometry");
 
@@ -74,24 +77,36 @@
   }
 }
 
-template <int DT, int KERNEL, bool PAIR>
-__global__ void __launch_bounds__(128)
+template <int DT, int KERNEL, bool PAIR, bool CHAIN>
+__global__ void __launch_bounds__(CHAIN ? KSTAR_CHAIN_THREADS : 128)
 cov_slices_kernel(const double* __restrict__ A, long long rows, int d, const double* __restrict__ Xt, int N, int Np,
                   const double* __restrict__ par, double inv_tau, const double* __restrict__ alpha, int8_t* __restrict__ ksS,
-                  double* __restrict__ meanP) {
+                  double* __restrict__ meanP, int* __restrict__ work) {
   __shared__ __align__(16) double s_x[DT][64];
   __shared__ double s_w[DT];
   __shared__ double s_tab[64];
-  __shared__ __align__(16) double s_al[64];
-  __shared__ double s_dot[64];
+  __shared__ __align__(16) double s_al[CHAIN ? 2 : 64];
+  __shared__ double s_dot[CHAIN ? 1 : 64];
+  __shared__ int s_item;
+  constexpr int NT = CHAIN ? KSTAR_CHAIN_THREADS : 128;
   if (threadIdx.x < 64) s_tab[threadIdx.x] = c_exp_tab[threadIdx.x];
-  const int ct = blockIdx.x, kb64 = blockIdx.y, KS_ALL = Np / KB;
+  const int n_ct = CHAIN ? (int)((rows + TN - 1) / TN) : (int)gridDim.x, KS_ALL = Np / KB;
+  for (;;) {
+  int ct = blockIdx.x, kb64 = blockIdx.y;
+  if (CHAIN) {
+    if (threadIdx.x == 0) s_item = atomicAdd(work, 1);
+    __syncthreads();
+    const int item = s_item;
+    if (item >= n_ct * (Np / 64)) break;
+    ct = item % n_ct;
+    kb64 = item / n_ct;
+  }
   const int c = threadIdx.x & 63;
-  for (int e = threadIdx.x; e < DT * 64; e += 128) {
+  for (int e = threadIdx.x; e < DT * 64; e += NT) {
     const int i = e / 64, k = kb64 * 64 + e % 64;
     s_x[i][e % 64] = (i < d && k < N) ? Xt[(long long)i * Np + k] : 0.0;
   }
-  if (threadIdx.x >= 64) s_al[c] = alpha[kb64 * 64 + c];
+  if (!CHAIN && threadIdx.x >= 64) s_al[c] = alpha[kb64 * 64 + c];
   if (threadIdx.x < DT) s_w[threadIdx.x] = threadIdx.x < d ? par[threadIdx.x] : 0.0;
   __syncthreads();
   const long long row = (long long)ct * TN + c;
@@ -99,7 +114,7 @@
 #pragma unroll
   for (int i = 0; i < DT; ++i) a[i] = (row < rows && i < d) ? A[row * d + i] : 0.0;
   const double sf2s = par[B7_MAX_DIMS] * inv_tau * 18014398509481984.0;
-  double dot = 0.0;
+  double dot = 0.0, dot_b = 0.0;
   double w[DT];
 #pragma unroll
   for (int j = 0; j < DT; ++j) w[j] = s_w[j];
@@ -107,8 +122,8 @@
   K.init();
   const bool live = row < rows;
 #pragma unroll 1
-  for (int half = 0; half < 2; ++half) {
-  const int kc = (threadIdx.x >> 6) + 2 * half;
+  for (int half = 0; half < (CHAIN ? 4 : 2); ++half) {
+  const int kc = CHAIN ? half : (threadIdx.x >> 6) + 2 * half;
   uint32_t pk[4][NS];
   unsigned long long z[4];
 #pragma unroll
@@ -133,7 +148,7 @@
     }
     va = (live && k < N) ? va : 0.0;
     vb = (live && k + 1 < N) ? vb : 0.0;
-    const double2 al = *reinterpret_cast<const double2*>(&s_al[kk]);
+    const double2 al = CHAIN ? __ldg(reinterpret_cast<const double2*>(alpha + kb64 * 64 + kk)) : *reinterpret_cast<const double2*>(&s_al[kk]);
     dot = fma(va, al.x, dot);
     dot = fma(vb, al.y, dot);
     z[i & 3] = digit_bytes_scaled(va);
@@ -146,10 +161,18 @@
   constexpr int P_STRIDE = PAIR ? KC * TNH * 16 : KC * TN * 16;
 #pragma unroll
   for (int p = 0; p < NS; ++p) *reinterpret_cast<uint4*>(dst + p * P_STRIDE) = make_uint4(pk[0][p], pk[1][p], pk[2][p], pk[3][p]);
+  if (CHAIN) { const double t = dot; dot = dot_b; dot_b = t; }
+  }
+  if (CHAIN) {
+    meanP[((long long)ct * (Np / 64) + kb64) * 64 + c] = dot + dot_b;
+    continue;
   }
   if (threadIdx.x >= 64) s_dot[c] = dot;
   __syncthreads();
   if (threadIdx.x < 64) meanP[((long long)ct * (Np / 64) + kb64) * 64 + c] = dot + s_dot[c];
+  break;
+  }
+  if (CHAIN) pdl_wait();
 }
 
 __device__ __forceinline__ double lane_transpose_sum(double (&x)[32], int lane) {
@@ -277,6 +300,7 @@
   __syncthreads();
   tc_fence_after();
   const uint32_t tmem = *tmem_slot;
+  pdl_trigger();
 
   if (warp == 4) {
     int slot = 0;
@@ -369,6 +393,7 @@
   cluster_sync_all();
   tc_fence_after();
   const uint32_t tmem = *tmem_slot;
+  pdl_trigger();
 
   if (warp == 8) {
     const uint64_t pol_last = l2_policy_evict_last(), pol_first = l2_policy_evict_first();
@@ -534,29 +559,25 @@
   return 0;
 }
 
+namespace {
+
+using CovSlicesFn = void (*)(const double*, long long, int, const double*, int, int, const double*, double, const double*, int8_t*, double*, int*);
+template <int DT, bool CHAIN>
+CovSlicesFn cov_slices_form(bool se, bool pair) {
+  if (pair) return se ? cov_slices_kernel<DT, B7_KERNEL_ARDSE, true, CHAIN> : cov_slices_kernel<DT, B7_KERNEL_MATERN52, true, CHAIN>;
+  return se ? cov_slices_kernel<DT, B7_KERNEL_ARDSE, false, CHAIN> : cov_slices_kernel<DT, B7_KERNEL_MATERN52, false, CHAIN>;
+}
 template <int DT>
-static int launch_cov_slices(b7_ctx* ctx, cudaStream_t st, int kernel, const double* A, int64_t rows, int64_t rows_pad, int d,
-                             const double* Xt, int N, int Np, const double* par, double inv_tau, const double* alpha, int8_t* ksS,
-                             double* meanP) {
-  dim3 grid((unsigned)(rows_pad / TN), Np / 64);
-  const bool se = kernel == B7_KERNEL_ARDSE;
-  if (ctx->post_pair) {
-    if (se) cov_slices_kernel<DT, B7_KERNEL_ARDSE, true><<<grid, 128, 0, st>>>(A, rows, d, Xt, N, Np, par, inv_tau, alpha, ksS, meanP);
-    else cov_slices_kernel<DT, B7_KERNEL_MATERN52, true><<<grid, 128, 0, st>>>(A, rows, d, Xt, N, Np, par, inv_tau, alpha, ksS, meanP);
+CovSlicesFn cov_slices_form(bool se, bool pair, bool chain) {
+  if constexpr (DT <= 8) {
+    if (chain) return cov_slices_form<DT, true>(se, pair);
   } else {
-    if (se) cov_slices_kernel<DT, B7_KERNEL_ARDSE, false><<<grid, 128, 0, st>>>(A, rows, d, Xt, N, Np, par, inv_tau, alpha, ksS, meanP);
-    else cov_slices_kernel<DT, B7_KERNEL_MATERN52, false><<<grid, 128, 0, st>>>(A, rows, d, Xt, N, Np, par, inv_tau, alpha, ksS, meanP);
-  }
-  b7_count(ctx);
-  B7_CUDA(cudaGetLastError());
-  return 0;
-}
-
-int b7_i8_cov_slices(b7_ctx* ctx, cudaStream_t st, int kernel, const double* A, int64_t rows, int64_t rows_pad, int d, const double* Xt,
-                     int N, int Np, const double* par, double tau, const double* alpha, int8_t* ksS, double* meanP) {
-  if (rows_pad <= 0) return 0;
-  const double inv_tau = 1.0 / tau;
-#define B7_COV_SLICES(DT) return launch_cov_slices<DT>(ctx, st, kernel, A, rows, rows_pad, d, Xt, N, Np, par, inv_tau, alpha, ksS, meanP)
+    if (chain) return nullptr;
+  }
+  return cov_slices_form<DT, false>(se, pair);
+}
+CovSlicesFn cov_slices_fn(int d, bool se, bool pair, bool chain) {
+#define B7_COV_SLICES(DT) return cov_slices_form<DT>(se, pair, chain)
   if (d <= 2) B7_COV_SLICES(2);
   if (d <= 4) B7_COV_SLICES(4);
   if (d <= 6) B7_COV_SLICES(6);
@@ -570,14 +591,78 @@
 #undef B7_COV_SLICES
 }
 
+std::unordered_map<const void*, signed char> g_kstar_state[16];
+
+int kstar_setup(b7_ctx* ctx, CovSlicesFn fn, bool chain, bool* fits) {
+  *fits = false;
+  if (!fn) return 0;
+  signed char& st = g_kstar_state[ctx->device & 15][(const void*)fn];
+  if (st == 0) {
+    B7_CUDA(cudaFuncSetAttribute((const void*)fn, cudaFuncAttributePreferredSharedMemoryCarveout, cudaSharedmemCarveoutMaxShared));
+    bool ok = true;
+    if (chain) {
+      const void* post = ctx->post_pair ? (const void*)posterior_i8_pair_kernel : (const void*)posterior_i8_kernel;
+      const int post_threads = ctx->post_pair ? P_THREADS : I8_THREADS, post_dyn = ctx->post_pair ? P_SMEM : I8_SMEM;
+      cudaFuncAttributes a, b;
+      B7_CUDA(cudaFuncGetAttributes(&a, post));
+      B7_CUDA(cudaFuncGetAttributes(&b, (const void*)fn));
+      int regs_sm = 0, smem_sm = 0, reserved = 0;
+      B7_CUDA(cudaDeviceGetAttribute(&regs_sm, cudaDevAttrMaxRegistersPerMultiprocessor, ctx->device));
+      B7_CUDA(cudaDeviceGetAttribute(&smem_sm, cudaDevAttrMaxSharedMemoryPerMultiprocessor, ctx->device));
+      B7_CUDA(cudaDeviceGetAttribute(&reserved, cudaDevAttrReservedSharedMemoryPerBlock, ctx->device));
+      auto warp_regs = [](int r) { return (r * 32 + 255) / 256 * 256; };
+      auto block_smem = [&](size_t bytes) { return (bytes + 127) / 128 * 128 + (size_t)reserved; };
+      const int post_warps = post_threads / 32, part_regs = regs_sm / 4;
+      const int light = 4 - post_warps % 4;
+      const int free_light = part_regs - post_warps / 4 * warp_regs(a.numRegs);
+      const size_t smem = block_smem(a.sharedSizeBytes + (size_t)post_dyn) + block_smem(b.sharedSizeBytes);
+      ok = KSTAR_CHAIN_THREADS / 32 <= light && warp_regs(b.numRegs) <= free_light && smem <= (size_t)smem_sm;
+    }
+    st = ok ? 1 : -1;
+  }
+  *fits = st > 0;
+  return 0;
+}
+
+}
+
+bool b7_i8_kstar_chains(b7_ctx* ctx, int kernel, int d) {
+  bool fits = false;
+  if (kstar_setup(ctx, cov_slices_fn(d, kernel == B7_KERNEL_ARDSE, ctx->post_pair, true), true, &fits) < 0) {
+    cudaGetLastError();
+    return false;
+  }
+  return fits;
+}
+
+int b7_i8_cov_slices(b7_ctx* ctx, int kernel, const double* A, int64_t rows, int64_t rows_pad, int d, const double* Xt,
+                     int N, int Np, const double* par, double tau, const double* alpha, int8_t* ksS, double* meanP, int* work) {
+  if (rows_pad <= 0) return 0;
+  const bool chain = work != nullptr;
+  const CovSlicesFn fn = cov_slices_fn(d, kernel == B7_KERNEL_ARDSE, ctx->post_pair, chain);
+  bool fits = false;
+  B7_CHECK(kstar_setup(ctx, fn, chain, &fits));
+  if (!fits) { b7_set_error("cov_slices: no chained K* pass fits beside the posterior pass at d = %d", d); return B7_ERR_ARG; }
+  const double inv_tau = 1.0 / tau;
+  if (chain) {
+    const int64_t n_items = rows_pad / TN * (Np / 64), grid = n_items < 12LL * ctx->sm_count ? n_items : 12LL * ctx->sm_count;
+    B7_CUDA(launch_pdl(fn, dim3((unsigned)grid), dim3(KSTAR_CHAIN_THREADS), 0, ctx->stream, true, A, (long long)rows, d, Xt, N, Np, par, inv_tau, alpha, ksS,
+                       meanP, work));
+  } else {
+    fn<<<dim3((unsigned)(rows_pad / TN), Np / 64), 128, 0, ctx->stream>>>(A, rows, d, Xt, N, Np, par, inv_tau, alpha, ksS, meanP, nullptr);
+  }
+  b7_count(ctx);
+  B7_CUDA(cudaGetLastError());
+  return 0;
+}
+
 size_t b7_i8_partial_bytes(int Np, int64_t cols_pad) {
   return (size_t)(cols_pad / TN) * ((size_t)(Np / TM) * TN + (size_t)(Np / 64) * 64) * sizeof(double);
 }
 double* b7_i8_mean_partials(double* partial, int Np, int64_t cols_pad) { return partial + (size_t)(cols_pad / TN) * (Np / TM) * TN; }
 
-int b7_launch_posterior_i8(b7_ctx* ctx, const int8_t* facS, const double* sigma, int Np, const int8_t* ksS, const double* cand,
-                           int64_t rows, int d, const double* Xt, const double* par, int kernel, int64_t cols_pad, double tau,
-                           double sf2, double mconst, double* partial, double* mean, double* var) {
+int b7_launch_posterior_i8(b7_ctx* ctx, const int8_t* facS, const double* sigma, int Np, const int8_t* ksS, int64_t cols_pad, double tau,
+                           double* partial) {
   if (!g_attr_i8[ctx->device & 15]) {
     B7_CUDA(cudaFuncSetAttribute(posterior_i8_kernel, cudaFuncAttributeMaxDynamicSharedMemorySize, I8_SMEM));
     B7_CUDA(cudaFuncSetAttribute(posterior_i8_pair_kernel, cudaFuncAttributeMaxDynamicSharedMemorySize, P_SMEM));
@@ -600,10 +685,19 @@
     posterior_i8_kernel<<<n_items < ctx->sm_count ? n_items : ctx->sm_count, I8_THREADS, I8_SMEM, ctx->stream>>>(facS, sigma, Np, NB, ksS, tau, chunk,
                                                                                                                 group, n_tiles, partial);
   }
-  posterior_i8_finish_kernel<<<(unsigned)((cols_pad + 127) / 128), 128, 0, ctx->stream>>>(partial, b7_i8_mean_partials(partial, Np, cols_pad), NB, Np,
-                                                                                         cand, rows, d, Xt, par, kernel, sf2, mconst,
-                                                                                         tau * 5.5511151231257827e-17, cols_pad, mean, var);
-  b7_count(ctx, 2);
+  b7_count(ctx);
   B7_CUDA(cudaGetLastError());
   return 0;
 }
+
+int b7_launch_posterior_i8_finish(b7_ctx* ctx, int Np, const double* cand, int64_t rows, int d, const double* Xt, const double* par,
+                                  int kernel, int64_t cols_pad, double tau, double sf2, double mconst, const double* partial, double* mean,
+                                  double* var) {
+  if (cols_pad <= 0) return 0;
+  posterior_i8_finish_kernel<<<(unsigned)((cols_pad + 127) / 128), 128, 0, ctx->stream>>>(
+      partial, b7_i8_mean_partials(const_cast<double*>(partial), Np, cols_pad), Np / TM, Np, cand, rows, d, Xt, par, kernel, sf2, mconst,
+      tau * 5.5511151231257827e-17, cols_pad, mean, var);
+  b7_count(ctx);
+  B7_CUDA(cudaGetLastError());
+  return 0;
+}
diff --git a/bot7_b200/csrc/potrf.cu b/bot7_b200/csrc/potrf.cu
--- a/bot7_b200/csrc/potrf.cu
+++ b/bot7_b200/csrc/potrf.cu
@@ -38,9 +38,6 @@
 #else
 #define DIAG_STAMP(i) do { } while (0)
 #endif
-
-__device__ __forceinline__ void pdl_wait() { asm volatile("griddepcontrol.wait;" ::: "memory"); }
-__device__ __forceinline__ void pdl_trigger() { asm volatile("griddepcontrol.launch_dependents;" ::: "memory"); }
 
 constexpr int BAR_S1 = 1, BAR_U = 2, BAR_S2 = 3;
 constexpr int UPD_THREADS = (DIAG_WARPS - DIAG_WARPS / 4) * 32;
@@ -752,25 +749,6 @@
   return 0;
 }
 
-template <typename... KArgs, typename... Args>
-cudaError_t launch_pdl(void (*kernel)(KArgs...), dim3 grid, dim3 block, size_t smem, cudaStream_t st, bool pdl, Args... args) {
-  cudaLaunchConfig_t cfg = {};
-  cfg.gridDim = grid;
-  cfg.blockDim = block;
-  cfg.dynamicSmemBytes = smem;
-  cfg.stream = st;
-  int prio = 0;
-  cudaStreamGetPriority(st, &prio);
-  cudaLaunchAttribute attr[2];
-  attr[0].id = cudaLaunchAttributePriority;
-  attr[0].val.priority = prio;
-  attr[1].id = cudaLaunchAttributeProgrammaticStreamSerialization;
-  attr[1].val.programmaticStreamSerializationAllowed = 1;
-  cfg.attrs = attr;
-  cfg.numAttrs = pdl ? 2 : 1;
-  return cudaLaunchKernelEx(&cfg, kernel, KArgs(args)...);
-}
-
 int potrf_latency_enqueue(b7_gp* gp, int s0, int count, int W, bool allow_trace) {
   b7_ctx* ctx = gp->ctx;
   static const bool pdl = !(getenv("B7_POTRF_PDL") && atoi(getenv("B7_POTRF_PDL")) == 0);
```

Result: slower. 169,500 (median of 6 runs) (-9.5%).
